# balaji1312/cassnat_asr_public

Measured on AMD Instinct MI355X. Metric: utterances_per_sec, higher is better.
Workload: dtype bf16; 1 GPU; BASELINE configs[1]: CASS-NAT 12L-enc / 1+3+2 dec blocks, d_model 256, 4 heads, d_ff 2048, V 5000, greedy NAST; 32 utterances x 1000 frames x 80 fbank per GPU per step; batch_per_gpu=32, frames=1000, feat_dim=80, global_batch=32, parallelism=utterance-sharded x1, decode_pipelines_per_gpu=2, batches_per_engine_pass=10, utterances_per_engine_pass=320, row_predictions=208, row_predictions_missed=0

## Files before the change

### cassnat_asr_public_amd/csrc/chain.hip

```cpp
#include <cstdio>
#include <cstdlib>
#include <algorithm>
#include <cmath>
#include <cstring>
#include <vector>

#include "kernels.h"

constexpr int CH_D = 256;
constexpr int CH_UNIT_BYTES = 16384;
constexpr int CH_RING = 8;
constexpr int CH_TAB_FLOATS = 5120;
constexpr int CH_TAB_BYTES = CH_TAB_FLOATS * 4;
constexpr int CH_LDS = CH_TAB_BYTES + CH_RING * CH_UNIT_BYTES;
static_assert(CH_LDS <= 160 * 1024, "LDS budget");
constexpr int CT_BO = 0, CT_LN1A = 256, CT_LN1B = 512, CT_B2 = 768, CT_NLNA = 1024, CT_NLNB = 1280, CT_BT = 1536,
              CT_B1 = 3072;
constexpr int CH_MAX_TAIL = 48, CH_MAX_FFN_TILES = 64;

__device__ long long ch_stamps[16];

typedef unsigned u32x4 __attribute__((ext_vector_type(4)));
typedef int v4i __attribute__((ext_vector_type(4)));
typedef int v8i __attribute__((ext_vector_type(8)));

struct ChainParams {
    float* x;
    const bf16* ctx;
    int ldctx;
    const uint4* wstream;
    const float* tab;
    bf16* out;
    int ldo;
    bf16* ln_out;
    int ld_ln;
    int M, ffn_tiles, tail_tiles, has_next;
    float eps;
    int stamps;
    int stamp_block;
    int x_in_blk, x_out_blk, store_x;
    int out_blk;
    int ctx_blk;
    const int* f8_q;
};

#define CH_STR2(x) #x
#define CH_STR(x) CH_STR2(x)
#define CH_DMA(src, dst)                                                                              \
    __builtin_amdgcn_global_load_lds((const __attribute__((address_space(1))) void*)(src),          \
                                     (__attribute__((address_space(3))) void*)(dst), 16, 0, 0)
#define CH_READ8(F, addr, OFFK)                                                                       \
    asm volatile("ds_read_b128 %0, %8 offset:" CH_STR(((OFFK) + 0) * 1024) "\n\t"                     \
                 "ds_read_b128 %1, %8 offset:" CH_STR(((OFFK) + 1) * 1024) "\n\t"                     \
                 "ds_read_b128 %2, %8 offset:" CH_STR(((OFFK) + 2) * 1024) "\n\t"                     \
                 "ds_read_b128 %3, %8 offset:" CH_STR(((OFFK) + 3) * 1024) "\n\t"                     \
                 "ds_read_b128 %4, %8 offset:" CH_STR(((OFFK) + 4) * 1024) "\n\t"                     \
                 "ds_read_b128 %5, %8 offset:" CH_STR(((OFFK) + 5) * 1024) "\n\t"                     \
                 "ds_read_b128 %6, %8 offset:" CH_STR(((OFFK) + 6) * 1024) "\n\t"                     \
                 "ds_read_b128 %7, %8 offset:" CH_STR(((OFFK) + 7) * 1024)                            \
                 : "=&v"(F[0]), "=&v"(F[1]), "=&v"(F[2]), "=&v"(F[3]), "=&v"(F[4]), "=&v"(F[5]),      \
                   "=&v"(F[6]), "=&v"(F[7])                                                           \
                 : "v"(addr)                                                                          \
                 : "memory")
#define CH_WAIT8(F)                                                                                   \
    asm volatile("s_waitcnt lgkmcnt(0)"                                                               \
                 : "+v"(F[0]), "+v"(F[1]), "+v"(F[2]), "+v"(F[3]), "+v"(F[4]), "+v"(F[5]), "+v"(F[6]), "+v"(F[7]) \
                 :: "memory")
__device__ __forceinline__ void ch_tab4_nowait(unsigned addr, f32x4& a, f32x4& b, f32x4& c, f32x4& d) {
    asm volatile("ds_read_b128 %0, %4\n\t"
                 "ds_read_b128 %1, %4 offset:32\n\t"
                 "ds_read_b128 %2, %4 offset:64\n\t"
                 "ds_read_b128 %3, %4 offset:96"
                 : "=&v"(a), "=&v"(b), "=&v"(c), "=&v"(d)
                 : "v"(addr)
                 : "memory");
}
template <typename D>
__device__ __forceinline__ void ch_tab4_nowait_after(unsigned addr, const D& dep, f32x4& a, f32x4& b, f32x4& c, f32x4& d) {
    asm volatile("ds_read_b128 %0, %4\n\t"
                 "ds_read_b128 %1, %4 offset:32\n\t"
                 "ds_read_b128 %2, %4 offset:64\n\t"
                 "ds_read_b128 %3, %4 offset:96"
                 : "=&v"(a), "=&v"(b), "=&v"(c), "=&v"(d)
                 : "v"(addr), "v"(dep)
                 : "memory");
}
template <typename D>
__device__ __forceinline__ void ch_tab4(unsigned addr, const D& dep, f32x4& a, f32x4& b, f32x4& c, f32x4& d) {
    asm volatile("ds_read_b128 %0, %4\n\t"
                 "ds_read_b128 %1, %4 offset:32\n\t"
                 "ds_read_b128 %2, %4 offset:64\n\t"
                 "ds_read_b128 %3, %4 offset:96\n\t"
                 "s_waitcnt lgkmcnt(0)"
                 : "=&v"(a), "=&v"(b), "=&v"(c), "=&v"(d)
                 : "v"(addr), "v"(dep)
                 : "memory");
}

#define CH_SB0_ __builtin_amdgcn_sched_barrier(0)
#define CH_LGKM_WAIT4(N, a, b, c, d) asm volatile("s_waitcnt lgkmcnt(" #N ")" : "+v"(a), "+v"(b), "+v"(c), "+v"(d) :: "memory")

template <bool ADD>
__device__ __forceinline__ void ch_layernorm_pack(f32x16 (&acc)[8], unsigned tab_lane, int off_a, int off_b, int off_add,
                                                  float eps, bf16x8 (&bop)[16]) {
    float s = 0.f;
#pragma unroll
    for (int nt = 0; nt < 8; ++nt)
#pragma unroll
        for (int r = 0; r < 16; ++r) s += acc[nt][r];
    s += __shfl_xor(s, 32);
    const float mean = s / (float)CH_D;
    float ss = 0.f;
#pragma unroll
    for (int nt = 0; nt < 8; ++nt)
#pragma unroll
        for (int r = 0; r < 16; ++r) ss = fmaf(acc[nt][r] - mean, acc[nt][r] - mean, ss);
    ss += __shfl_xor(ss, 32);
    const float inv = 1.0f / (sqrtf(ss / (float)(CH_D - 1)) + eps);
    f32x4 ga[2][4], be[2][4], ad[2][4];
    CH_SB0_;
    ch_tab4_nowait_after(tab_lane + off_a * 4, inv, ga[0][0], ga[0][1], ga[0][2], ga[0][3]);
    ch_tab4_nowait(tab_lane + off_b * 4, be[0][0], be[0][1], be[0][2], be[0][3]);
    if constexpr (ADD) ch_tab4_nowait(tab_lane + off_add * 4, ad[0][0], ad[0][1], ad[0][2], ad[0][3]);
#pragma unroll
    for (int nt = 0; nt < 8; ++nt) {
        const int c = nt & 1, n = c ^ 1;
        if (nt + 1 < 8) {
            ch_tab4_nowait(tab_lane + (off_a + 32 * (nt + 1)) * 4, ga[n][0], ga[n][1], ga[n][2], ga[n][3]);
            ch_tab4_nowait(tab_lane + (off_b + 32 * (nt + 1)) * 4, be[n][0], be[n][1], be[n][2], be[n][3]);
            if constexpr (ADD) ch_tab4_nowait(tab_lane + (off_add + 32 * (nt + 1)) * 4, ad[n][0], ad[n][1], ad[n][2], ad[n][3]);
            if constexpr (ADD) {
                CH_LGKM_WAIT4(12, ga[c][0], ga[c][1], ga[c][2], ga[c][3]);
                CH_LGKM_WAIT4(12, be[c][0], be[c][1], be[c][2], be[c][3]);
                CH_LGKM_WAIT4(12, ad[c][0], ad[c][1], ad[c][2], ad[c][3]);
            } else {
                CH_LGKM_WAIT4(8, ga[c][0], ga[c][1], ga[c][2], ga[c][3]);
                CH_LGKM_WAIT4(8, be[c][0], be[c][1], be[c][2], be[c][3]);
            }
        } else {
            CH_LGKM_WAIT4(0, ga[c][0], ga[c][1], ga[c][2], ga[c][3]);
            CH_LGKM_WAIT4(0, be[c][0], be[c][1], be[c][2], be[c][3]);
            if constexpr (ADD) CH_LGKM_WAIT4(0, ad[c][0], ad[c][1], ad[c][2], ad[c][3]);
        }
#pragma unroll
        for (int g = 0; g < 4; ++g)
#pragma unroll
            for (int e = 0; e < 4; ++e) {
                const int r = 4 * g + e;
                bop[2 * nt + (r >> 3)][r & 7] = (bf16)fmaf(ga[c][g][e] * (acc[nt][r] - mean), inv, be[c][g][e]);
                if constexpr (ADD) acc[nt][r] += ad[c][g][e];
            }
        asm volatile("" : "+v"(bop[2 * nt]), "+v"(bop[2 * nt + 1]));
        if constexpr (ADD) asm volatile("" : "+a"(acc[nt]));
    }
}

__device__ __forceinline__ void ch_add_channel(f32x16 (&acc)[8], unsigned tab_lane, int off) {
    f32x4 b[2][4];
    ch_tab4_nowait(tab_lane + off * 4, b[0][0], b[0][1], b[0][2], b[0][3]);
#pragma unroll
    for (int nt = 0; nt < 8; ++nt) {
        const int c = nt & 1, n = c ^ 1;
        if (nt + 1 < 8) {
            ch_tab4_nowait(tab_lane + (off + 32 * (nt + 1)) * 4, b[n][0], b[n][1], b[n][2], b[n][3]);
            CH_LGKM_WAIT4(4, b[c][0], b[c][1], b[c][2], b[c][3]);
        } else {
            CH_LGKM_WAIT4(0, b[c][0], b[c][1], b[c][2], b[c][3]);
        }
#pragma unroll
        for (int g = 0; g < 4; ++g)
#pragma unroll
            for (int e = 0; e < 4; ++e) acc[nt][4 * g + e] += b[c][g][e];
        asm volatile("" : "+a"(acc[nt]));
    }
}

template <int XS, int CS, bool CTX>
__device__ __forceinline__ void ch_load_rows(f32x4 (&xr)[32], bf16x8 (&bop)[16], const float* const (&xb)[8], const bf16* const (&cb)[4]) {
    if constexpr (CTX) {
        asm volatile("global_load_dwordx4 %[x0], %[xb0], off\n\t"
                     "global_load_dwordx4 %[x1], %[xb0], off offset:%[xo1]\n\t"
                     "global_load_dwordx4 %[x2], %[xb0], off offset:%[xo2]\n\t"
                     "global_load_dwordx4 %[x3], %[xb0], off offset:%[xo3]\n\t"
                     "global_load_dwordx4 %[x4], %[xb1], off\n\t"
                     "global_load_dwordx4 %[x5], %[xb1], off offset:%[xo1]\n\t"
                     "global_load_dwordx4 %[x6], %[xb1], off offset:%[xo2]\n\t"
                     "global_load_dwordx4 %[x7], %[xb1], off offset:%[xo3]\n\t"
                     "global_load_dwordx4 %[x8], %[xb2], off\n\t"
                     "global_load_dwordx4 %[x9], %[xb2], off offset:%[xo1]\n\t"
                     "global_load_dwordx4 %[x10], %[xb2], off offset:%[xo2]\n\t"
                     "global_load_dwordx4 %[x11], %[xb2], off offset:%[xo3]\n\t"
                     "global_load_dwordx4 %[x12], %[xb3], off\n\t"
                     "global_load_dwordx4 %[x13], %[xb3], off offset:%[xo1]\n\t"
                     "global_load_dwordx4 %[x14], %[xb3], off offset:%[xo2]\n\t"
                     "global_load_dwordx4 %[x15], %[xb3], off offset:%[xo3]\n\t"
                     "global_load_dwordx4 %[x16], %[xb4], off\n\t"
                     "global_load_dwordx4 %[x17], %[xb4], off offset:%[xo1]\n\t"
                     "global_load_dwordx4 %[x18], %[xb4], off offset:%[xo2]\n\t"
                     "global_load_dwordx4 %[x19], %[xb4], off offset:%[xo3]\n\t"
                     "global_load_dwordx4 %[x20], %[xb5], off\n\t"
                     "global_load_dwordx4 %[x21], %[xb5], off offset:%[xo1]\n\t"
                     "global_load_dwordx4 %[x22], %[xb5], off offset:%[xo2]\n\t"
                     "global_load_dwordx4 %[x23], %[xb5], off offset:%[xo3]\n\t"
                     "global_load_dwordx4 %[x24], %[xb6], off\n\t"
                     "global_load_dwordx4 %[x25], %[xb6], off offset:%[xo1]\n\t"
                     "global_load_dwordx4 %[x26], %[xb6], off offset:%[xo2]\n\t"
                     "global_load_dwordx4 %[x27], %[xb6], off offset:%[xo3]\n\t"
                     "global_load_dwordx4 %[x28], %[xb7], off\n\t"
                     "global_load_dwordx4 %[x29], %[xb7], off offset:%[xo1]\n\t"
                     "global_load_dwordx4 %[x30], %[xb7], off offset:%[xo2]\n\t"
                     "global_load_dwordx4 %[x31], %[xb7], off offset:%[xo3]\n\t"
                     "global_load_dwordx4 %[c0], %[cb0], off\n\t"
                     "global_load_dwordx4 %[c1], %[cb0], off offset:%[co1]\n\t"
                     "global_load_dwordx4 %[c2], %[cb0], off offset:%[co2]\n\t"
                     "global_load_dwordx4 %[c3], %[cb0], off offset:%[co3]\n\t"
                     "global_load_dwordx4 %[c4], %[cb1], off\n\t"
                     "global_load_dwordx4 %[c5], %[cb1], off offset:%[co1]\n\t"
                     "global_load_dwordx4 %[c6], %[cb1], off offset:%[co2]\n\t"
                     "global_load_dwordx4 %[c7], %[cb1], off offset:%[co3]\n\t"
                     "global_load_dwordx4 %[c8], %[cb2], off\n\t"
                     "global_load_dwordx4 %[c9], %[cb2], off offset:%[co1]\n\t"
                     "global_load_dwordx4 %[c10], %[cb2], off offset:%[co2]\n\t"
                     "global_load_dwordx4 %[c11], %[cb2], off offset:%[co3]\n\t"
                     "global_load_dwordx4 %[c12], %[cb3], off\n\t"
                     "global_load_dwordx4 %[c13], %[cb3], off offset:%[co1]\n\t"
                     "global_load_dwordx4 %[c14], %[cb3], off offset:%[co2]\n\t"
                     "global_load_dwordx4 %[c15], %[cb3], off offset:%[co3]\n\t"
                     "s_waitcnt vmcnt(0)"
                     : [x0] "=&a"(xr[0]), [x1] "=&a"(xr[1]), [x2] "=&a"(xr[2]), [x3] "=&a"(xr[3]), [x4] "=&a"(xr[4]), [x5] "=&a"(xr[5]), [x6] "=&a"(xr[6]), [x7] "=&a"(xr[7]), [x8] "=&a"(xr[8]), [x9] "=&a"(xr[9]), [x10] "=&a"(xr[10]), [x11] "=&a"(xr[11]), [x12] "=&a"(xr[12]), [x13] "=&a"(xr[13]), [x14] "=&a"(xr[14]), [x15] "=&a"(xr[15]), [x16] "=&a"(xr[16]), [x17] "=&a"(xr[17]), [x18] "=&a"(xr[18]), [x19] "=&a"(xr[19]), [x20] "=&a"(xr[20]), [x21] "=&a"(xr[21]), [x22] "=&a"(xr[22]), [x23] "=&a"(xr[23]), [x24] "=&a"(xr[24]), [x25] "=&a"(xr[25]), [x26] "=&a"(xr[26]), [x27] "=&a"(xr[27]), [x28] "=&a"(xr[28]), [x29] "=&a"(xr[29]), [x30] "=&a"(xr[30]), [x31] "=&a"(xr[31]), [c0] "=&v"(bop[0]), [c1] "=&v"(bop[1]), [c2] "=&v"(bop[2]), [c3] "=&v"(bop[3]), [c4] "=&v"(bop[4]), [c5] "=&v"(bop[5]), [c6] "=&v"(bop[6]), [c7] "=&v"(bop[7]), [c8] "=&v"(bop[8]), [c9] "=&v"(bop[9]), [c10] "=&v"(bop[10]), [c11] "=&v"(bop[11]), [c12] "=&v"(bop[12]), [c13] "=&v"(bop[13]), [c14] "=&v"(bop[14]), [c15] "=&v"(bop[15])
                     : [xb0] "v"(xb[0]), [xb1] "v"(xb[1]), [xb2] "v"(xb[2]), [xb3] "v"(xb[3]), [xb4] "v"(xb[4]), [xb5] "v"(xb[5]), [xb6] "v"(xb[6]), [xb7] "v"(xb[7]), [cb0] "v"(cb[0]), [cb1] "v"(cb[1]), [cb2] "v"(cb[2]), [cb3] "v"(cb[3])
                       , [xo1] "n"(XS), [xo2] "n"(2 * XS), [xo3] "n"(3 * XS), [co1] "n"(CS), [co2] "n"(2 * CS), [co3] "n"(3 * CS)
                     : "memory");
    } else {
        asm volatile("global_load_dwordx4 %[x0], %[xb0], off\n\t"
                     "global_load_dwordx4 %[x1], %[xb0], off offset:%[xo1]\n\t"
                     "global_load_dwordx4 %[x2], %[xb0], off offset:%[xo2]\n\t"
                     "global_load_dwordx4 %[x3], %[xb0], off offset:%[xo3]\n\t"
                     "global_load_dwordx4 %[x4], %[xb1], off\n\t"
                     "global_load_dwordx4 %[x5], %[xb1], off offset:%[xo1]\n\t"
                     "global_load_dwordx4 %[x6], %[xb1], off offset:%[xo2]\n\t"
                     "global_load_dwordx4 %[x7], %[xb1], off offset:%[xo3]\n\t"
                     "global_load_dwordx4 %[x8], %[xb2], off\n\t"
                     "global_load_dwordx4 %[x9], %[xb2], off offset:%[xo1]\n\t"
                     "global_load_dwordx4 %[x10], %[xb2], off offset:%[xo2]\n\t"
                     "global_load_dwordx4 %[x11], %[xb2], off offset:%[xo3]\n\t"
                     "global_load_dwordx4 %[x12], %[xb3], off\n\t"
                     "global_load_dwordx4 %[x13], %[xb3], off offset:%[xo1]\n\t"
                     "global_load_dwordx4 %[x14], %[xb3], off offset:%[xo2]\n\t"
                     "global_load_dwordx4 %[x15], %[xb3], off offset:%[xo3]\n\t"
                     "global_load_dwordx4 %[x16], %[xb4], off\n\t"
                     "global_load_dwordx4 %[x17], %[xb4], off offset:%[xo1]\n\t"
                     "global_load_dwordx4 %[x18], %[xb4], off offset:%[xo2]\n\t"
                     "global_load_dwordx4 %[x19], %[xb4], off offset:%[xo3]\n\t"
                     "global_load_dwordx4 %[x20], %[xb5], off\n\t"
                     "global_load_dwordx4 %[x21], %[xb5], off offset:%[xo1]\n\t"
                     "global_load_dwordx4 %[x22], %[xb5], off offset:%[xo2]\n\t"
                     "global_load_dwordx4 %[x23], %[xb5], off offset:%[xo3]\n\t"
                     "global_load_dwordx4 %[x24], %[xb6], off\n\t"
                     "global_load_dwordx4 %[x25], %[xb6], off offset:%[xo1]\n\t"
                     "global_load_dwordx4 %[x26], %[xb6], off offset:%[xo2]\n\t"
                     "global_load_dwordx4 %[x27], %[xb6], off offset:%[xo3]\n\t"
                     "global_load_dwordx4 %[x28], %[xb7], off\n\t"
                     "global_load_dwordx4 %[x29], %[xb7], off offset:%[xo1]\n\t"
                     "global_load_dwordx4 %[x30], %[xb7], off offset:%[xo2]\n\t"
                     "global_load_dwordx4 %[x31], %[xb7], off offset:%[xo3]\n\t"
                     "s_waitcnt vmcnt(0)"
                     : [x0] "=&a"(xr[0]), [x1] "=&a"(xr[1]), [x2] "=&a"(xr[2]), [x3] "=&a"(xr[3]), [x4] "=&a"(xr[4]), [x5] "=&a"(xr[5]), [x6] "=&a"(xr[6]), [x7] "=&a"(xr[7]), [x8] "=&a"(xr[8]), [x9] "=&a"(xr[9]), [x10] "=&a"(xr[10]), [x11] "=&a"(xr[11]), [x12] "=&a"(xr[12]), [x13] "=&a"(xr[13]), [x14] "=&a"(xr[14]), [x15] "=&a"(xr[15]), [x16] "=&a"(xr[16]), [x17] "=&a"(xr[17]), [x18] "=&a"(xr[18]), [x19] "=&a"(xr[19]), [x20] "=&a"(xr[20]), [x21] "=&a"(xr[21]), [x22] "=&a"(xr[22]), [x23] "=&a"(xr[23]), [x24] "=&a"(xr[24]), [x25] "=&a"(xr[25]), [x26] "=&a"(xr[26]), [x27] "=&a"(xr[27]), [x28] "=&a"(xr[28]), [x29] "=&a"(xr[29]), [x30] "=&a"(xr[30]), [x31] "=&a"(xr[31])
                     : [xb0] "v"(xb[0]), [xb1] "v"(xb[1]), [xb2] "v"(xb[2]), [xb3] "v"(xb[3]), [xb4] "v"(xb[4]), [xb5] "v"(xb[5]), [xb6] "v"(xb[6]), [xb7] "v"(xb[7])
                       , [xo1] "n"(XS), [xo2] "n"(2 * XS), [xo3] "n"(3 * XS)
                     : "memory");
    }
}

__device__ __forceinline__ void ch_layernorm_pack8(f32x16 (&acc)[8], unsigned tab_lane, int off_a, int off_b, int off_add,
                                                   float eps, v4i (&b8)[8]) {
    float s = 0.f;
#pragma unroll
    for (int nt = 0; nt < 8; ++nt)
#pragma unroll
        for (int r = 0; r < 16; ++r) s += acc[nt][r];
    s += __shfl_xor(s, 32);
    const float mean = s / (float)CH_D;
    float ss = 0.f;
#pragma unroll
    for (int nt = 0; nt < 8; ++nt)
#pragma unroll
        for (int r = 0; r < 16; ++r) ss = fmaf(acc[nt][r] - mean, acc[nt][r] - mean, ss);
    ss += __shfl_xor(ss, 32);
    const float inv = 1.0f / (sqrtf(ss / (float)(CH_D - 1)) + eps);
    f32x4 ga[2][4], be[2][4], ad[2][4];
    CH_SB0_;
    ch_tab4_nowait_after(tab_lane + off_a * 4, inv, ga[0][0], ga[0][1], ga[0][2], ga[0][3]);
    ch_tab4_nowait(tab_lane + off_b * 4, be[0][0], be[0][1], be[0][2], be[0][3]);
    ch_tab4_nowait(tab_lane + off_add * 4, ad[0][0], ad[0][1], ad[0][2], ad[0][3]);
#pragma unroll
    for (int nt = 0; nt < 8; ++nt) {
        const int c = nt & 1, n = c ^ 1;
        if (nt + 1 < 8) {
            ch_tab4_nowait(tab_lane + (off_a + 32 * (nt + 1)) * 4, ga[n][0], ga[n][1], ga[n][2], ga[n][3]);
            ch_tab4_nowait(tab_lane + (off_b + 32 * (nt + 1)) * 4, be[n][0], be[n][1], be[n][2], be[n][3]);
            ch_tab4_nowait(tab_lane + (off_add + 32 * (nt + 1)) * 4, ad[n][0], ad[n][1], ad[n][2], ad[n][3]);
            CH_LGKM_WAIT4(12, ga[c][0], ga[c][1], ga[c][2], ga[c][3]);
            CH_LGKM_WAIT4(12, be[c][0], be[c][1], be[c][2], be[c][3]);
            CH_LGKM_WAIT4(12, ad[c][0], ad[c][1], ad[c][2], ad[c][3]);
        } else {
            CH_LGKM_WAIT4(0, ga[c][0], ga[c][1], ga[c][2], ga[c][3]);
            CH_LGKM_WAIT4(0, be[c][0], be[c][1], be[c][2], be[c][3]);
            CH_LGKM_WAIT4(0, ad[c][0], ad[c][1], ad[c][2], ad[c][3]);
        }
#pragma unroll
        for (int g = 0; g < 4; ++g) {
            float v[4];
#pragma unroll
            for (int e = 0; e < 4; ++e) {
                v[e] = __builtin_amdgcn_fmed3f(fmaf(ga[c][g][e] * (acc[nt][4 * g + e] - mean), inv, be[c][g][e]), -448.f, 448.f);
                acc[nt][4 * g + e] += ad[c][g][e];
            }
            b8[nt][g] = __builtin_amdgcn_cvt_pk_fp8_f32(v[0], v[1], b8[nt][g], false);
            b8[nt][g] = __builtin_amdgcn_cvt_pk_fp8_f32(v[2], v[3], b8[nt][g], true);
        }
        asm volatile("" : "+v"(b8[nt]));
        asm volatile("" : "+a"(acc[nt]));
    }
}

#define CH_LAND_FRAGMENTS(EXTRA)                                                                                \
    asm volatile(EXTRA "s_waitcnt lgkmcnt(0)"                                                                  \
                 : "+v"(Fa[0]), "+v"(Fa[1]), "+v"(Fa[2]), "+v"(Fa[3]), "+v"(Fa[4]), "+v"(Fa[5]), "+v"(Fa[6]), "+v"(Fa[7]),     \
                   "+v"(Fb[0]), "+v"(Fb[1]), "+v"(Fb[2]), "+v"(Fb[3]), "+v"(Fb[4]), "+v"(Fb[5]), "+v"(Fb[6]), "+v"(Fb[7])      \
                 :: "memory")

#define CH_MF CN_MFMA16_ASM
#define CH_DRAIN "s_nop 13\n\t"
#define CH_NODRAIN ""
#ifdef CH_EXP_NO_READ
#define CH_RD2(n0, n1, K) ""
#else
#define CH_RD2(n0, n1, K) "ds_read_b128 %[" #n0 "], %[ra] offset:" CH_STR((K) * 1024) "\n\t"                   \
                          "ds_read_b128 %[" #n1 "], %[ra] offset:" CH_STR(((K) + 1) * 1024) "\n\t"
#endif
#define CH_PRE_A "s_waitcnt lgkmcnt(0)\n\t"
#define CH_PRE_A4 "s_waitcnt lgkmcnt(4)\n\t"
#define CH_PRE_BO(M0OFF) "s_add_u32 m0, %[m0w], " CH_STR(M0OFF) "\n\ts_waitcnt lgkmcnt(0)\n\t"
#ifdef CH_EXP_NO_BARRIER
#define CH_PRE_BE(M0OFF) CH_PRE_BO(M0OFF)
#else
#define CH_PRE_BE(M0OFF) "s_waitcnt vmcnt(16)\n\ts_barrier\n\ts_add_u32 m0, %[m0w], " CH_STR(M0OFF) "\n\ts_waitcnt lgkmcnt(0)\n\t"
#endif
#define CH_PRE_B_0 CH_PRE_BE
#define CH_PRE_B_1 CH_PRE_BO
#define CH_PRE_B_2 CH_PRE_BE
#define CH_PRE_B_3 CH_PRE_BO
#define CH_PRE_B_4 CH_PRE_BE
#define CH_PRE_B_5 CH_PRE_BO
#define CH_PRE_B_6 CH_PRE_BE
#define CH_PRE_B_7 CH_PRE_BO
#ifdef CH_EXP_NO_DMA
#define CH_DMA0(SOFF) "v_add_u32 %[tv], " CH_STR(SOFF) ", %[vo]\n\t"
#define CH_DMA1 ""
#define CH_DMA2 ""
#define CH_DMA3 ""
#else
#define CH_DMA0(SOFF) "v_add_u32 %[tv], " CH_STR(SOFF) ", %[vo]\n\tglobal_load_lds_dwordx4 %[tv], %[sb]\n\t"
#define CH_DMA1 "global_load_lds_dwordx4 %[tv], %[sb] offset:1024\n\t"
#define CH_DMA2 "global_load_lds_dwordx4 %[tv], %[sb] offset:2048\n\t"
#define CH_DMA3 "global_load_lds_dwordx4 %[tv], %[sb] offset:3072\n\t"
#endif
#define CH_BLK1(CIO, CC, C0, acc, Fc, B, BO, Fn, RA, RK, PRE, D0, D1, D2, D3, SB, POST)                        \
    asm volatile(PRE                                                                                           \
                 CH_MF "%[c], %[f0], %[b0], " C0 "\n\t" CH_RD2(n0, n1, (RK) + 0)                               \
                 CH_MF "%[c], %[f1], %[b1], %[c]\n\t" CH_RD2(n2, n3, (RK) + 2)                                 \
                 CH_MF "%[c], %[f2], %[b2], %[c]\n\t" CH_RD2(n4, n5, (RK) + 4)                                 \
                 CH_MF "%[c], %[f3], %[b3], %[c]\n\t" CH_RD2(n6, n7, (RK) + 6)                                 \
                 CH_MF "%[c], %[f4], %[b4], %[c]\n\t" D0                                                       \
                 CH_MF "%[c], %[f5], %[b5], %[c]\n\t" D1                                                       \
                 CH_MF "%[c], %[f6], %[b6], %[c]\n\t" D2                                                       \
                 CH_MF "%[c], %[f7], %[b7], %[c]\n\t" D3 POST                                                  \
                 : [c] CIO CC(acc), [n0] "=&v"(Fn[0]), [n1] "=&v"(Fn[1]), [n2] "=&v"(Fn[2]), [n3] "=&v"(Fn[3]), \
                   [n4] "=&v"(Fn[4]), [n5] "=&v"(Fn[5]), [n6] "=&v"(Fn[6]), [n7] "=&v"(Fn[7]), [tv] "=&v"(tv)  \
                 : [f0] "v"(Fc[0]), [f1] "v"(Fc[1]), [f2] "v"(Fc[2]), [f3] "v"(Fc[3]), [f4] "v"(Fc[4]),        \
                   [f5] "v"(Fc[5]), [f6] "v"(Fc[6]), [f7] "v"(Fc[7]), [b0] "v"(B[(BO) + 0]), [b1] "v"(B[(BO) + 1]), \
                   [b2] "v"(B[(BO) + 2]), [b3] "v"(B[(BO) + 3]), [b4] "v"(B[(BO) + 4]), [b5] "v"(B[(BO) + 5]), \
                   [b6] "v"(B[(BO) + 6]), [b7] "v"(B[(BO) + 7]), [ra] "v"(RA), [m0w] "s"(m0_wave), [vo] "v"(voff), \
                   [sb] "s"(SB)                                                                                \
                 : "memory", "scc")
#define CH_BLK1A(K, acc, Fc, B, BO, Fn, RA, RK, PRE, D0, D1, D2, D3, SB, POST)                                 \
    asm volatile(PRE                                                                                           \
                 CH_MF "%[c" #K "], %[f0], %[b0], %[c" #K "]\n\t" CH_RD2(n0, n1, (RK) + 0)                       \
                 CH_MF "%[c" #K "], %[f1], %[b1], %[c" #K "]\n\t" CH_RD2(n2, n3, (RK) + 2)                       \
                 CH_MF "%[c" #K "], %[f2], %[b2], %[c" #K "]\n\t" CH_RD2(n4, n5, (RK) + 4)                       \
                 CH_MF "%[c" #K "], %[f3], %[b3], %[c" #K "]\n\t" CH_RD2(n6, n7, (RK) + 6)                       \
                 CH_MF "%[c" #K "], %[f4], %[b4], %[c" #K "]\n\t" D0                                           \
                 CH_MF "%[c" #K "], %[f5], %[b5], %[c" #K "]\n\t" D1                                           \
                 CH_MF "%[c" #K "], %[f6], %[b6], %[c" #K "]\n\t" D2                                           \
                 CH_MF "%[c" #K "], %[f7], %[b7], %[c" #K "]\n\t" D3 POST                                      \
                 : [c0] "+a"(acc[0]), [c1] "+a"(acc[1]), [c2] "+a"(acc[2]), [c3] "+a"(acc[3]), [c4] "+a"(acc[4]), \
                   [c5] "+a"(acc[5]), [c6] "+a"(acc[6]), [c7] "+a"(acc[7]), [n0] "=&v"(Fn[0]), [n1] "=&v"(Fn[1]), \
                   [n2] "=&v"(Fn[2]), [n3] "=&v"(Fn[3]), [n4] "=&v"(Fn[4]), [n5] "=&v"(Fn[5]), [n6] "=&v"(Fn[6]), \
                   [n7] "=&v"(Fn[7]), [tv] "=&v"(tv)                                                           \
                 : [f0] "v"(Fc[0]), [f1] "v"(Fc[1]), [f2] "v"(Fc[2]), [f3] "v"(Fc[3]), [f4] "v"(Fc[4]),        \
                   [f5] "v"(Fc[5]), [f6] "v"(Fc[6]), [f7] "v"(Fc[7]), [b0] "v"(B[(BO) + 0]), [b1] "v"(B[(BO) + 1]), \
                   [b2] "v"(B[(BO) + 2]), [b3] "v"(B[(BO) + 3]), [b4] "v"(B[(BO) + 4]), [b5] "v"(B[(BO) + 5]), \
                   [b6] "v"(B[(BO) + 6]), [b7] "v"(B[(BO) + 7]), [ra] "v"(RA), [m0w] "s"(m0_wave), [vo] "v"(voff), \
                   [sb] "s"(SB)                                                                                \
                 : "memory", "scc")
#define CH_BLK2(acc, Fc, pbv, Fn, RA, RK, PRE, D0, D1, D2, D3, SB, POST)                                       \
    asm volatile(PRE                                                                                           \
                 CH_MF "%[c0], %[f0], %[pb], %[c0]\n\t" CH_RD2(n0, n1, (RK) + 0)                               \
                 CH_MF "%[c1], %[f1], %[pb], %[c1]\n\t" CH_RD2(n2, n3, (RK) + 2)                               \
                 CH_MF "%[c2], %[f2], %[pb], %[c2]\n\t" CH_RD2(n4, n5, (RK) + 4)                               \
                 CH_MF "%[c3], %[f3], %[pb], %[c3]\n\t" CH_RD2(n6, n7, (RK) + 6)                               \
                 CH_MF "%[c4], %[f4], %[pb], %[c4]\n\t" D0                                                     \
                 CH_MF "%[c5], %[f5], %[pb], %[c5]\n\t" D1                                                     \
                 CH_MF "%[c6], %[f6], %[pb], %[c6]\n\t" D2                                                     \
                 CH_MF "%[c7], %[f7], %[pb], %[c7]\n\t" D3 POST                                                \
                 : [c0] "+a"(acc[0]), [c1] "+a"(acc[1]), [c2] "+a"(acc[2]), [c3] "+a"(acc[3]), [c4] "+a"(acc[4]), \
                   [c5] "+a"(acc[5]), [c6] "+a"(acc[6]), [c7] "+a"(acc[7]), [n0] "=&v"(Fn[0]), [n1] "=&v"(Fn[1]), \
                   [n2] "=&v"(Fn[2]), [n3] "=&v"(Fn[3]), [n4] "=&v"(Fn[4]), [n5] "=&v"(Fn[5]), [n6] "=&v"(Fn[6]), \
                   [n7] "=&v"(Fn[7]), [tv] "=&v"(tv)                                                           \
                 : [f0] "v"(Fc[0]), [f1] "v"(Fc[1]), [f2] "v"(Fc[2]), [f3] "v"(Fc[3]), [f4] "v"(Fc[4]),        \
                   [f5] "v"(Fc[5]), [f6] "v"(Fc[6]), [f7] "v"(Fc[7]), [pb] "v"(pbv), [ra] "v"(RA),             \
                   [m0w] "s"(m0_wave), [vo] "v"(voff), [sb] "s"(SB)                                            \
                 : "memory", "scc")
#define CH_M1R(PRE, X, F, B, N0, N1, RA, K)                                                                    \
    asm volatile(PRE CH_MF "%[c], %[f], %[b], %[c]\n\t" CH_RD2(n0, n1, K)                                      \
                 : [c] "+v"(X), [n0] "=&v"(N0), [n1] "=&v"(N1)                                                 \
                 : [f] "v"(F), [b] "v"(B), [ra] "v"(RA)                                                        \
                 : "memory")
#define CH_M1(X, F, B) asm volatile(CH_MF "%[c], %[f], %[b], %[c]" : [c] "+v"(X) : [f] "v"(F), [b] "v"(B) : "memory")
#define CH_SB0 __builtin_amdgcn_sched_barrier(0)

#define CH8_MF "v_mfma_scale_f32_32x32x64_f8f6f4 "
#define CH8_SC ", %[qa], %[qb] op_sel_hi:[0,0,0]\n\t"
#define CH8_DRAIN "s_nop 15\n\ts_nop 4\n\t"
#define CH8_JOIN(lo, hi) __builtin_shufflevector(__builtin_bit_cast(v4i, lo), __builtin_bit_cast(v4i, hi), 0, 1, 2, 3, 4, 5, 6, 7)
#define CH8_A(F, t) CH8_JOIN(F[2 * (t)], F[2 * (t) + 1])
#define CH8_M1R(PRE, X, A, B, N0, N1, N2, N3, RA, K, QA, QB)                                                   \
    asm volatile(PRE CH8_MF "%[c], %[a], %[b], %[c]" CH8_SC CH_RD2(n0, n1, K) CH_RD2(n2, n3, (K) + 2)          \
                 : [c] "+v"(X), [n0] "=&v"(N0), [n1] "=&v"(N1), [n2] "=&v"(N2), [n3] "=&v"(N3)                 \
                 : [a] "v"(A), [b] "v"(B), [ra] "v"(RA), [qa] "v"(QA), [qb] "v"(QB), [m0w] "s"(m0_wave)         \
                 : "memory", "scc")
#define CH8_M1(X, A, B, QA, QB)                                                                                \
    asm volatile(CH8_MF "%[c], %[a], %[b], %[c]" CH8_SC : [c] "+v"(X) : [a] "v"(A), [b] "v"(B), [qa] "v"(QA), [qb] "v"(QB) : "memory")
#define CH8_M1D(M0OFF, X, A, B, D0, D1, SB, QA, QB)                                                            \
    asm volatile("s_add_u32 m0, %[m0w], " CH_STR(M0OFF) "\n\t" CH8_MF "%[c], %[a], %[b], %[c]" CH8_SC D0 D1    \
                 : [c] "+v"(X), [tv] "+v"(tv)                                                                  \
                 : [a] "v"(A), [b] "v"(B), [qa] "v"(QA), [qb] "v"(QB), [vo] "v"(voff), [sb] "s"(SB),            \
                   [m0w] "s"(m0_wave)                                                                          \
                 : "memory", "scc")
#define CH8_BLK2(acc, C0, C1, C2, C3, A0, A1, A2, A3, HB, Fn, RA, RK, PRE, D0, D1, D2, D3, SB, POST, QA, QB)    \
    asm volatile(PRE                                                                                           \
                 CH8_MF "%[" #C0 "], %[a0], %[hb], %[" #C0 "]" CH8_SC CH_RD2(n0, n1, (RK) + 0) CH_RD2(n2, n3, (RK) + 2) \
                 CH8_MF "%[" #C1 "], %[a1], %[hb], %[" #C1 "]" CH8_SC CH_RD2(n4, n5, (RK) + 4) CH_RD2(n6, n7, (RK) + 6) \
                 CH8_MF "%[" #C2 "], %[a2], %[hb], %[" #C2 "]" CH8_SC D0 D1                                    \
                 CH8_MF "%[" #C3 "], %[a3], %[hb], %[" #C3 "]" CH8_SC D2 D3 POST                               \
                 : [c0] "+a"(acc[0]), [c1] "+a"(acc[1]), [c2] "+a"(acc[2]), [c3] "+a"(acc[3]), [c4] "+a"(acc[4]), \
                   [c5] "+a"(acc[5]), [c6] "+a"(acc[6]), [c7] "+a"(acc[7]), [n0] "=&v"(Fn[0]), [n1] "=&v"(Fn[1]), \
                   [n2] "=&v"(Fn[2]), [n3] "=&v"(Fn[3]), [n4] "=&v"(Fn[4]), [n5] "=&v"(Fn[5]), [n6] "=&v"(Fn[6]), \
                   [n7] "=&v"(Fn[7]), [tv] "=&v"(tv)                                                           \
                 : [a0] "v"(A0), [a1] "v"(A1), [a2] "v"(A2), [a3] "v"(A3), [hb] "v"(HB), [ra] "v"(RA),         \
                   [m0w] "s"(m0_wave), [vo] "v"(voff), [sb] "s"(SB), [qa] "v"(QA), [qb] "v"(QB)                \
                 : "memory", "scc")

#define CH_POSITIONS(X)                                                                                        \
    X(0, ra0, 8, ra0, 16, 0x1C000, 0x1C000, sb_cur)  X(1, ra0, 24, ra0, 32, 0x0, 0x0, sb_next)                 \
    X(2, ra0, 40, ra0, 48, 0x4000, 0x4000, sb_next)  X(3, ra0, 56, ra1, 0, 0x8000, 0x8000, sb_next)            \
    X(4, ra1, 8, ra1, 16, 0xC000, 0xC000, sb_next)   X(5, ra1, 24, ra1, 32, 0x10000, 0x10000, sb_next)         \
    X(6, ra1, 40, ra1, 48, 0x14000, 0x14000, sb_next) X(7, ra1, 56, ra0, 0, 0x18000, 0x18000, sb_next)

template <bool SWISH, bool F8>
__global__ __launch_bounds__(256) void chain_kernel(ChainParams p) {
    extern __shared__ __attribute__((aligned(16))) unsigned char smem[];
    const int tid = threadIdx.x, lane = tid & 63;
    const int wave = __builtin_amdgcn_readfirstlane(tid >> 6);
    const int half = lane >> 5, l31 = lane & 31;
    const int m = blockIdx.x * 128 + 32 * wave + l31;
    const int mc = m < p.M ? m : p.M - 1;
    const bool live = m < p.M;
#define CH_STAMP(i)                                                                              \
    if (p.stamps && (int)blockIdx.x == p.stamp_block && tid == 0) ch_stamps[i] = (long long)__builtin_amdgcn_s_memtime();
    CH_STAMP(0)
    if (p.stamps && (int)blockIdx.x == p.stamp_block && tid == 0) ch_stamps[10] = (long long)__builtin_amdgcn_s_memrealtime();
    const int G_OUT = p.ctx ? 1 : 0, G_FFN = F8 ? p.ffn_tiles >> 3 : p.ffn_tiles >> 2, G_TAIL = p.tail_tiles >> 3;
    const int NG = G_OUT + G_FFN + G_TAIL;
#ifdef CH_ROTATE
    const int rotg = G_FFN ? (int)((blockIdx.x * 5u) % (unsigned)G_FFN) : 0;
#else
    const int rotg = 0;
#endif
    unsigned char* ring = smem + CH_TAB_BYTES;
    auto ffn_group = [&](int g) -> int { return g + rotg >= G_FFN ? g + rotg - G_FFN : g + rotg; };
    auto group_base = [&](int g) -> const uint4* {
        if (g > NG - 1) g = NG - 1;
        if (g >= G_OUT && g < G_OUT + G_FFN) g = G_OUT + ffn_group(g - G_OUT);
        return p.wstream + (long long)g * 8 * 1024;
    };

    f32x4 xr[32];
    bf16x8 bop[16];
    const int rb = blockIdx.x * 4 + wave, nrb = (p.M + 31) >> 5;
    {
        const uint4* ts = reinterpret_cast<const uint4*>(p.tab) + 5 * wave * 64 + lane;
#pragma unroll
        for (int j = 0; j < 5; ++j) CH_DMA(ts + j * 64, smem + (5 * wave + j) * 1024);
    }
    if (NG > 0) {
        const uint4* g0 = group_base(0);
        for (int u = 0; u < CH_RING - 1; ++u) {
            const uint4* src = g0 + ((long long)u * 16 + 4 * wave) * 64 + lane;
            unsigned char* dst = ring + u * CH_UNIT_BYTES + 4 * wave * 1024;
#pragma unroll
            for (int j = 0; j < 4; ++j) CH_DMA(src + j * 64, dst + j * 1024);
        }
    }
    {
#ifdef CH_EXP_HOT_X
        const float* xp = p.x + (long long)wave * 8192 + 4 * lane;
#else
        const float* xp = p.x_in_blk ? p.x + (long long)(rb < nrb ? rb : nrb - 1) * 8192 + 4 * lane
                                     : p.x + (long long)mc * CH_D + 4 * half;
#endif
        const int step = p.x_in_blk ? 256 : 8;
        const float* xb[8];
#pragma unroll
        for (int nt = 0; nt < 8; ++nt) xb[nt] = xp + step * 4 * nt;
        const bf16* cp = !p.ctx ? nullptr
                         : p.ctx_blk ? p.ctx + ((long long)(rb < nrb ? rb : nrb - 1) * 16 * 64 + lane) * 8
                                     : p.ctx + (long long)mc * p.ldctx + 8 * half;
        const int cstep = p.ctx_blk ? 512 : 16;
        const bf16* cb[4];
#pragma unroll
        for (int q = 0; q < 4; ++q) cb[q] = cp + cstep * 4 * q;
        if (!p.ctx) {
            if (p.x_in_blk) ch_load_rows<1024, 32, false>(xr, bop, xb, cb);
            else ch_load_rows<32, 32, false>(xr, bop, xb, cb);
        } else if (p.x_in_blk) {
            if (p.ctx_blk) ch_load_rows<1024, 1024, true>(xr, bop, xb, cb);
            else ch_load_rows<1024, 32, true>(xr, bop, xb, cb);
        } else {
            if (p.ctx_blk) ch_load_rows<32, 1024, true>(xr, bop, xb, cb);
            else ch_load_rows<32, 32, true>(xr, bop, xb, cb);
        }
    }

    f32x16 acc[8];
#pragma unroll
    for (int nt = 0; nt < 8; ++nt)
#pragma unroll
        for (int g = 0; g < 4; ++g)
#pragma unroll
            for (int e = 0; e < 4; ++e) acc[nt][4 * g + e] = xr[4 * nt + g][e];
    CH_STAMP(1)

    const unsigned ring_lds = (unsigned)(size_t)(__attribute__((address_space(3))) unsigned char*)ring;
    const unsigned ra0 = ring_lds + lane * 16, ra1 = ra0 + 4 * CH_UNIT_BYTES;
    const unsigned tab_lane = (unsigned)(size_t)(__attribute__((address_space(3))) unsigned char*)(smem + 16 * half);
    const unsigned voff = (unsigned)(lane * 16 + wave * 4096);
    const unsigned m0_wave = __builtin_amdgcn_readfirstlane(ring_lds + wave * 4096);
    unsigned tv = 0;

    bf16x8 Fa[8], Fb[8];
    asm volatile("s_waitcnt vmcnt(0)\n\ts_barrier" ::: "memory");
    CH_STAMP(2)
    int gpos = 0;

    if (p.ctx) {
        const uint4* sb_cur = group_base(gpos);
        const uint4* sb_next = group_base(gpos + 1);
#define CH_S1(k, RA_A, RK_A, RA_B, RK_B, M0OFF, SOFF, SB)                                                     \
        CH_BLK1A(k, acc, Fa, bop, 0, Fb, RA_A, RK_A, CH_PRE_A, "", "", "", "", SB, CH_NODRAIN);                \
        CH_BLK1A(k, acc, Fb, bop, 8, Fa, RA_B, RK_B, CH_PRE_B_##k(M0OFF), CH_DMA0(SOFF), CH_DMA1, CH_DMA2, CH_DMA3, SB, CH_NODRAIN);
        CH_READ8(Fa, ra0, 0);
        CH_WAIT8(Fa);
        asm volatile("s_nop 1" ::: "memory");
        CH_POSITIONS(CH_S1)
#undef CH_S1
        CH_LAND_FRAGMENTS("");
        asm volatile(CH_DRAIN : "+a"(acc[0]), "+a"(acc[1]), "+a"(acc[2]), "+a"(acc[3]), "+a"(acc[4]), "+a"(acc[5]),
                     "+a"(acc[6]), "+a"(acc[7]) :: "memory");
        ++gpos;
        ch_add_channel(acc, tab_lane, CT_BO);
    }
    CH_STAMP(3)

    if constexpr (F8) {
      if (p.ffn_tiles) {
        v4i b8[8] = {};
        ch_layernorm_pack8(acc, tab_lane, CT_LN1A, CT_LN1B, CT_B2, p.eps, b8);
        CH_STAMP(4)
        const int NP = p.ffn_tiles >> 1;
        f32x16 xa0, xb0, xa1, xb1;
        f32x4 b1v[8];
        v8i hid8 = {};
        const int qa1 = p.f8_q[0], qb1 = p.f8_q[1], qa2 = p.f8_q[2], qb2 = p.f8_q[3];
        auto tabp = [&](int pp) -> unsigned { return tab_lane + (unsigned)((CT_B1 + 64 * (pp < NP ? pp : NP - 1)) * 4); };
#define CH8_TAB8(addr)                                                                                         \
        ch_tab4_nowait(addr, b1v[0], b1v[1], b1v[2], b1v[3]);                                                  \
        ch_tab4_nowait((addr) + 128, b1v[4], b1v[5], b1v[6], b1v[7]);
#define CH8_B(kk) CH8_JOIN(b8[2 * (kk)], b8[2 * (kk) + 1])
        CH8_TAB8(tabp(0))
        CH_READ8(Fa, ra0, 0);
        asm volatile("s_waitcnt lgkmcnt(0)" : "+v"(b1v[0]), "+v"(b1v[1]), "+v"(b1v[2]), "+v"(b1v[3]), "+v"(b1v[4]), "+v"(b1v[5]),
                     "+v"(b1v[6]), "+v"(b1v[7]), "+v"(Fa[0]), "+v"(Fa[1]), "+v"(Fa[2]), "+v"(Fa[3]), "+v"(Fa[4]), "+v"(Fa[5]),
                     "+v"(Fa[6]), "+v"(Fa[7]) :: "memory");
#define CH8_ACT_PIECE(XA, XB, i)                                                                               \
        {                                                                                                      \
            const float v0_ = __builtin_amdgcn_fmed3f(((i) < 4 ? XA : XB)[4 * ((i) & 3) + 0], 0.f, 448.f);     \
            const float v1_ = __builtin_amdgcn_fmed3f(((i) < 4 ? XA : XB)[4 * ((i) & 3) + 1], 0.f, 448.f);     \
            const float v2_ = __builtin_amdgcn_fmed3f(((i) < 4 ? XA : XB)[4 * ((i) & 3) + 2], 0.f, 448.f);     \
            const float v3_ = __builtin_amdgcn_fmed3f(((i) < 4 ? XA : XB)[4 * ((i) & 3) + 3], 0.f, 448.f);     \
            hid8[i] = __builtin_amdgcn_cvt_pk_fp8_f32(v0_, v1_, hid8[i], false);                               \
            hid8[i] = __builtin_amdgcn_cvt_pk_fp8_f32(v2_, v3_, hid8[i], true);                                \
            asm volatile("" : "+v"(hid8));                                                                     \
        }
#define CH8_ACT_GAP(HAS_OLD, XA, XB, i)                                                                        \
        CH_SB0;                                                                                                \
        if constexpr (HAS_OLD) CH8_ACT_PIECE(XA, XB, i)                                                        \
        CH_SB0;
#define CH8_BIAS16(lo) __builtin_shufflevector(__builtin_shufflevector(b1v[lo], b1v[(lo) + 1], 0, 1, 2, 3, 4, 5, 6, 7),   \
                                               __builtin_shufflevector(b1v[(lo) + 2], b1v[(lo) + 3], 0, 1, 2, 3, 4, 5, 6, 7), \
                                               0, 1, 2, 3, 4, 5, 6, 7, 8, 9, 10, 11, 12, 13, 14, 15)
#define CH8_W1N(k, RA_A, RK_A, RA_B, RK_B, M0OFF, SOFF, SB, XNA, XNB, XOA, XOB, HAS_OLD, PNEXT)                 \
        XNA = CH8_BIAS16(0);                                                                                   \
        XNB = CH8_BIAS16(4);                                                                                   \
        CH8_M1R(CH_PRE_A, XNA, CH8_A(Fa, 0), CH8_B(0), Fb[0], Fb[1], Fb[2], Fb[3], RA_A, (RK_A) + 0, qa1, qb1); \
        CH8_ACT_GAP(HAS_OLD, XOA, XOB, 0)                                                                      \
        CH8_M1R("", XNA, CH8_A(Fa, 1), CH8_B(1), Fb[4], Fb[5], Fb[6], Fb[7], RA_A, (RK_A) + 4, qa1, qb1);      \
        CH8_ACT_GAP(HAS_OLD, XOA, XOB, 1)                                                                      \
        CH8_M1(XNA, CH8_A(Fa, 2), CH8_B(2), qa1, qb1);                                                         \
        CH8_ACT_GAP(HAS_OLD, XOA, XOB, 2)                                                                      \
        CH8_M1(XNA, CH8_A(Fa, 3), CH8_B(3), qa1, qb1);                                                         \
        CH8_ACT_GAP(HAS_OLD, XOA, XOB, 3)                                                                      \
        CH8_M1R(CH_PRE_B_##k(M0OFF), XNB, CH8_A(Fb, 0), CH8_B(0), Fa[0], Fa[1], Fa[2], Fa[3], RA_B, (RK_B) + 0, qa1, qb1); \
        CH8_ACT_GAP(HAS_OLD, XOA, XOB, 4)                                                                      \
        CH8_M1R("", XNB, CH8_A(Fb, 1), CH8_B(1), Fa[4], Fa[5], Fa[6], Fa[7], RA_B, (RK_B) + 4, qa1, qb1);      \
        CH8_ACT_GAP(HAS_OLD, XOA, XOB, 5)                                                                      \
        CH8_M1D(M0OFF, XNB, CH8_A(Fb, 2), CH8_B(2), CH_DMA0(SOFF), CH_DMA1, SB, qa1, qb1);                            \
        CH8_ACT_GAP(HAS_OLD, XOA, XOB, 6)                                                                      \
        CH8_M1D(M0OFF, XNB, CH8_A(Fb, 3), CH8_B(3), CH_DMA2, CH_DMA3, SB, qa1, qb1);                                  \
        CH8_ACT_GAP(HAS_OLD, XOA, XOB, 7)                                                                      \
        CH8_TAB8(tabp(PNEXT))
#define CH8_PRE_A8 "s_waitcnt lgkmcnt(8)\n\t"
#define CH8_W2N(k, RA_A, RK_A, RA_B, RK_B, M0OFF, SOFF, SB, PREA, POST)                                        \
        CH8_BLK2(acc, c0, c1, c2, c3, CH8_A(Fa, 0), CH8_A(Fa, 1), CH8_A(Fa, 2), CH8_A(Fa, 3), hid8, Fb, RA_A, RK_A, PREA, "", "", \
                 "", "", SB, CH_NODRAIN, qa2, qb2);                                                            \
        CH8_BLK2(acc, c4, c5, c6, c7, CH8_A(Fb, 0), CH8_A(Fb, 1), CH8_A(Fb, 2), CH8_A(Fb, 3), hid8, Fa, RA_B, RK_B,              \
                 CH_PRE_B_##k(M0OFF), CH_DMA0(SOFF), CH_DMA1, CH_DMA2, CH_DMA3, SB, POST, qa2, qb2);
#define CH8_FFN_GROUP(FIRST, LAST)                                                                             \
        {                                                                                                      \
            const uint4* sb_cur = group_base(gpos);                                                            \
            const uint4* sb_next = group_base(gpos + 1);                                                       \
            const int t0 = 4 * g;                                                                              \
            if constexpr (FIRST) {                                                                             \
                CH8_W1N(0, ra0, 8, ra0, 16, 0x1C000, 0x1C000, sb_cur, xa0, xb0, xa1, xb1, false, 1)            \
                             \
                asm volatile(CH8_DRAIN "s_waitcnt lgkmcnt(0)" : "+v"(xa0), "+v"(xb0), "+v"(b1v[0]), "+v"(b1v[1]), "+v"(b1v[2]), \
                             "+v"(b1v[3]), "+v"(b1v[4]), "+v"(b1v[5]), "+v"(b1v[6]), "+v"(b1v[7]), "+v"(Fa[0]), "+v"(Fa[1]),     \
                             "+v"(Fa[2]), "+v"(Fa[3]), "+v"(Fa[4]), "+v"(Fa[5]), "+v"(Fa[6]), "+v"(Fa[7]) :: "memory");          \
            } else {                                                                                           \
                CH8_W2N(0, ra0, 8, ra0, 16, 0x1C000, 0x1C000, sb_cur, CH8_PRE_A8, CH_NODRAIN)                  \
            }                                                                                                  \
            CH8_W1N(1, ra0, 24, ra0, 32, 0x0, 0x0, sb_next, xa1, xb1, xa0, xb0, true, t0 + 2)                  \
            CH8_W2N(2, ra0, 40, ra0, 48, 0x4000, 0x4000, sb_next, CH8_PRE_A8, CH_NODRAIN)                      \
            CH8_W1N(3, ra0, 56, ra1, 0, 0x8000, 0x8000, sb_next, xa0, xb0, xa1, xb1, true, t0 + 3)             \
            CH8_W2N(4, ra1, 8, ra1, 16, 0xC000, 0xC000, sb_next, CH8_PRE_A8, CH_NODRAIN)                       \
            CH8_W1N(5, ra1, 24, ra1, 32, 0x10000, 0x10000, sb_next, xa1, xb1, xa0, xb0, true, t0 + 4)          \
            CH8_W2N(6, ra1, 40, ra1, 48, 0x14000, 0x14000, sb_next, CH8_PRE_A8, CH_NODRAIN)                    \
            if constexpr (!(LAST)) {                                                                           \
                CH8_W1N(7, ra1, 56, ra0, 0, 0x18000, 0x18000, sb_next, xa0, xb0, xa1, xb1, true, t0 + 5)       \
            } else {                                                                                           \
                               \
                asm volatile("" : "+v"(xa1), "+v"(xb1));                                                       \
                CH_SB0;                                                                                        \
                CH8_ACT_PIECE(xa1, xb1, 0) CH8_ACT_PIECE(xa1, xb1, 1) CH8_ACT_PIECE(xa1, xb1, 2) CH8_ACT_PIECE(xa1, xb1, 3) \
                CH8_ACT_PIECE(xa1, xb1, 4) CH8_ACT_PIECE(xa1, xb1, 5) CH8_ACT_PIECE(xa1, xb1, 6) CH8_ACT_PIECE(xa1, xb1, 7) \
                CH_SB0;                                                                                        \
                CH8_W2N(7, ra1, 56, ra0, 0, 0x18000, 0x18000, sb_next, CH_PRE_A, CH8_DRAIN "s_waitcnt lgkmcnt(0)\n\t") \
            }                                                                                                  \
            ++g;                                                                                               \
            ++gpos;                                                                                            \
        }
        int g = 0;
        if (G_FFN == 1) {
            CH8_FFN_GROUP(true, true)
        } else {
            CH8_FFN_GROUP(true, false)
            while (g < G_FFN - 1) CH8_FFN_GROUP(false, false)
            CH8_FFN_GROUP(false, true)
        }
#undef CH8_FFN_GROUP
#undef CH8_W1N
#undef CH8_W2N
#undef CH8_ACT_GAP
#undef CH8_ACT_PIECE
        CH_LAND_FRAGMENTS("");
        asm volatile("s_waitcnt lgkmcnt(0)" : "+v"(b1v[0]), "+v"(b1v[1]), "+v"(b1v[2]), "+v"(b1v[3]), "+v"(b1v[4]), "+v"(b1v[5]),
                     "+v"(b1v[6]), "+v"(b1v[7]) :: "memory");
      }
    } else
    if (p.ffn_tiles) {
        ch_layernorm_pack<true>(acc, tab_lane, CT_LN1A, CT_LN1B, CT_B2, p.eps, bop);
        CH_STAMP(4)
        const int NTL = p.ffn_tiles;
        f32x16 xh0, xh1;
        f32x4 b1v[4];
        bf16x8 pb[2];
        auto tabb = [&](int t) -> unsigned { return tab_lane + (unsigned)((CT_B1 + 32 * (t < NTL ? t : NTL - 1)) * 4); };
        ch_tab4_nowait(tabb(0), b1v[0], b1v[1], b1v[2], b1v[3]);
        CH_READ8(Fa, ra0, 0);
        asm volatile("s_waitcnt lgkmcnt(0)" : "+v"(b1v[0]), "+v"(b1v[1]), "+v"(b1v[2]), "+v"(b1v[3]), "+v"(Fa[0]), "+v"(Fa[1]), "+v"(Fa[2]),
                     "+v"(Fa[3]), "+v"(Fa[4]), "+v"(Fa[5]), "+v"(Fa[6]), "+v"(Fa[7]) :: "memory");
#define CH_ACT_PIECE(XO, i)                                                                                    \
        {                                                                                                      \
            if constexpr (SWISH) {                                                                             \
                const float v0_ = XO[2 * (i)], v1_ = XO[2 * (i) + 1];                                          \
                pb[(i) >> 2][2 * ((i) & 3)] = (bf16)(v0_ * (1.f / (1.f + __expf(-v0_))));                      \
                pb[(i) >> 2][2 * ((i) & 3) + 1] = (bf16)(v1_ * (1.f / (1.f + __expf(-v1_))));                  \
            } else {                                                                                           \
                const int b0_ = __float_as_int(XO[2 * (i)]), b1_ = __float_as_int(XO[2 * (i) + 1]);            \
                pb[(i) >> 2][2 * ((i) & 3)] = (bf16)__int_as_float(b0_ > 0 ? b0_ : 0);                         \
                pb[(i) >> 2][2 * ((i) & 3) + 1] = (bf16)__int_as_float(b1_ > 0 ? b1_ : 0);                     \
            }                                                                                                  \
            asm volatile("" : "+v"(pb[(i) >> 2]));   \
        }
#define CH_ACT_GAP(HAS_OLD, XO, i)                                                                             \
        CH_SB0;                                                                                                \
        if constexpr (HAS_OLD) CH_ACT_PIECE(XO, i)                                                             \
        CH_SB0;
#define CH_W1N(k, RA_A, RK_A, RA_B, RK_B, M0OFF, SOFF, SB, XN, XO, HAS_OLD, TNEXT)                             \
        XN = __builtin_shufflevector(__builtin_shufflevector(b1v[0], b1v[1], 0, 1, 2, 3, 4, 5, 6, 7),          \
                                     __builtin_shufflevector(b1v[2], b1v[3], 0, 1, 2, 3, 4, 5, 6, 7),          \
                                     0, 1, 2, 3, 4, 5, 6, 7, 8, 9, 10, 11, 12, 13, 14, 15);                   \
        CH_M1R(CH_PRE_A, XN, Fa[0], bop[0], Fb[0], Fb[1], RA_A, (RK_A) + 0);                                   \
        CH_ACT_GAP(HAS_OLD, XO, 0)                                                                             \
        CH_M1R("", XN, Fa[1], bop[1], Fb[2], Fb[3], RA_A, (RK_A) + 2);                                         \
        CH_ACT_GAP(HAS_OLD, XO, 1)                                                                             \
        CH_M1R("", XN, Fa[2], bop[2], Fb[4], Fb[5], RA_A, (RK_A) + 4);                                         \
        CH_ACT_GAP(HAS_OLD, XO, 2)                                                                             \
        CH_M1R("", XN, Fa[3], bop[3], Fb[6], Fb[7], RA_A, (RK_A) + 6);                                         \
        CH_ACT_GAP(HAS_OLD, XO, 3)                                                                             \
        CH_M1(XN, Fa[4], bop[4]);                                                                              \
        CH_ACT_GAP(HAS_OLD, XO, 4)                                                                             \
        CH_M1(XN, Fa[5], bop[5]);                                                                              \
        CH_ACT_GAP(HAS_OLD, XO, 5)                                                                             \
        CH_M1(XN, Fa[6], bop[6]);                                                                              \
        CH_ACT_GAP(HAS_OLD, XO, 6)                                                                             \
        CH_M1(XN, Fa[7], bop[7]);                                                                              \
        CH_ACT_GAP(HAS_OLD, XO, 7)                                                                             \
        CH_BLK1("+", "v", "%[c]", XN, Fb, bop, 8, Fa, RA_B, RK_B, CH_PRE_B_##k(M0OFF), CH_DMA0(SOFF), CH_DMA1, CH_DMA2, \
                CH_DMA3, SB, CH_NODRAIN);                                                                      \
        ch_tab4_nowait(tabb(TNEXT), b1v[0], b1v[1], b1v[2], b1v[3]);
#define CH_W2N(k, RA_A, RK_A, RA_B, RK_B, M0OFF, SOFF, SB, PREA, POST)                                        \
        CH_BLK2(acc, Fa, pb[0], Fb, RA_A, RK_A, PREA, "", "", "", "", SB, CH_NODRAIN);                         \
        CH_BLK2(acc, Fb, pb[1], Fa, RA_B, RK_B, CH_PRE_B_##k(M0OFF), CH_DMA0(SOFF), CH_DMA1, CH_DMA2, CH_DMA3, SB, POST);
#define CH_FFN_GROUP(FIRST, LAST)                                                                              \
        {                                                                                                      \
            const uint4* sb_cur = group_base(gpos);                                                            \
            const uint4* sb_next = group_base(gpos + 1);                                                       \
            const int t0 = 4 * g;                                                                              \
            if constexpr (FIRST) {                                                                             \
                CH_W1N(0, ra0, 8, ra0, 16, 0x1C000, 0x1C000, sb_cur, xh0, xh1, false, 1)                       \
                 \
                 \
                 \
                asm volatile("s_nop 13\n\ts_nop 13\n\ts_waitcnt lgkmcnt(0)" : "+v"(xh0), "+v"(b1v[0]), "+v"(b1v[1]), "+v"(b1v[2]), "+v"(b1v[3]), "+v"(Fa[0]), \
                             "+v"(Fa[1]), "+v"(Fa[2]), "+v"(Fa[3]), "+v"(Fa[4]), "+v"(Fa[5]), "+v"(Fa[6]), "+v"(Fa[7]) :: "memory"); \
            } else {                                                                                           \
                CH_W2N(0, ra0, 8, ra0, 16, 0x1C000, 0x1C000, sb_cur, CH_PRE_A4, CH_NODRAIN)                    \
            }                                                                                                  \
            CH_W1N(1, ra0, 24, ra0, 32, 0x0, 0x0, sb_next, xh1, xh0, true, t0 + 2)                             \
            CH_W2N(2, ra0, 40, ra0, 48, 0x4000, 0x4000, sb_next, CH_PRE_A4, CH_NODRAIN)                        \
            CH_W1N(3, ra0, 56, ra1, 0, 0x8000, 0x8000, sb_next, xh0, xh1, true, t0 + 3)                        \
            CH_W2N(4, ra1, 8, ra1, 16, 0xC000, 0xC000, sb_next, CH_PRE_A4, CH_NODRAIN)                         \
            CH_W1N(5, ra1, 24, ra1, 32, 0x10000, 0x10000, sb_next, xh1, xh0, true, t0 + 4)                     \
            CH_W2N(6, ra1, 40, ra1, 48, 0x14000, 0x14000, sb_next, CH_PRE_A4, CH_NODRAIN)                      \
            if constexpr (!(LAST)) {                                                                           \
                CH_W1N(7, ra1, 56, ra0, 0, 0x18000, 0x18000, sb_next, xh0, xh1, true, t0 + 5)                  \
            } else {                                                                                           \
                 \
                 \
                 \
                asm volatile("" : "+v"(xh1));                                                                  \
                CH_SB0;                                                                                        \
                _Pragma("unroll") for (int i = 0; i < 8; ++i) CH_ACT_PIECE(xh1, i)                             \
                CH_SB0;                                                                                        \
                CH_W2N(7, ra1, 56, ra0, 0, 0x18000, 0x18000, sb_next, CH_PRE_A, CH_DRAIN "s_waitcnt lgkmcnt(0)\n\t") \
            }                                                                                                  \
            ++g;                                                                                               \
            ++gpos;                                                                                            \
        }
        int g = 0;
        if (G_FFN == 1) {
            CH_FFN_GROUP(true, true)
        } else {
            CH_FFN_GROUP(true, false)
            while (g < G_FFN - 1) CH_FFN_GROUP(false, false)
            CH_FFN_GROUP(false, true)
        }
#undef CH_FFN_GROUP
#undef CH_W1N
#undef CH_W2N
#undef CH_ACT_GAP
#undef CH_ACT_PIECE
        CH_LAND_FRAGMENTS("");
        asm volatile("s_waitcnt lgkmcnt(0)" : "+v"(b1v[0]), "+v"(b1v[1]), "+v"(b1v[2]), "+v"(b1v[3]) :: "memory");
    }
    CH_STAMP(5)

    if (p.store_x && (p.x_out_blk ? rb < nrb : live)) {
        float* xp = p.x_out_blk ? p.x + (long long)rb * 8192 + 4 * lane : p.x + (long long)m * CH_D + 4 * half;
        const int step = p.x_out_blk ? 256 : 8;
#pragma unroll
        for (int nt = 0; nt < 8; ++nt)
#pragma unroll
            for (int g = 0; g < 4; ++g) {
                f32x4 o;
#pragma unroll
                for (int e = 0; e < 4; ++e) o[e] = acc[nt][4 * g + e];
                *reinterpret_cast<f32x4*>(xp + step * (4 * nt + g)) = o;
            }
    }
    CH_STAMP(6)
    if (p.has_next) {
        ch_layernorm_pack<false>(acc, tab_lane, CT_NLNA, CT_NLNB, 0, p.eps, bop);
        CH_STAMP(7)
        if (p.ln_out) {
            if (live) {
                bf16* op = p.ln_out + (long long)m * p.ld_ln + 4 * half;
#pragma unroll
                for (int k = 0; k < 16; ++k)
#pragma unroll
                    for (int q = 0; q < 2; ++q) {
                        bf16x4 o;
#pragma unroll
                        for (int e = 0; e < 4; ++e) o[e] = bop[k][4 * q + e];
                        *reinterpret_cast<bf16x4*>(op + 16 * k + 8 * q) = o;
                    }
            }
        }
        if (G_TAIL > 0) {
            f32x16 q0, q1;
            f32x4 btv[4];
            bf16x4 o_[4];
            u32x4 w_[2];
            const int NTT = 8 * G_TAIL;
            auto tabt = [&](int tt) -> unsigned { return tab_lane + (unsigned)((CT_BT + 32 * (tt < NTT ? tt : NTT - 1)) * 4); };
            bf16* op16 = p.out + (long long)m * p.ldo + 8 * half;
            unsigned char* ob16 = reinterpret_cast<unsigned char*>(p.out) + (long long)rb * (p.ldo >> 5) * 2048 + lane * 16;
            unsigned char* st_base = p.out_blk ? ob16 : reinterpret_cast<unsigned char*>(op16);
            const int st_tile = p.out_blk ? 2048 : 64, st_half = p.out_blk ? 1024 : 32;
            const bool st_on = (p.out_blk ? rb < nrb : live) && p.stamps != 2;
            ch_tab4_nowait(tabt(0), btv[0], btv[1], btv[2], btv[3]);
            CH_READ8(Fa, ra0, 0);
            asm volatile("s_waitcnt lgkmcnt(0)" : "+v"(btv[0]), "+v"(btv[1]), "+v"(btv[2]), "+v"(btv[3]), "+v"(Fa[0]), "+v"(Fa[1]),
                         "+v"(Fa[2]), "+v"(Fa[3]), "+v"(Fa[4]), "+v"(Fa[5]), "+v"(Fa[6]), "+v"(Fa[7]) :: "memory");
#define CH_TAIL_STORE(v, ptr) *(ptr) = (v)
#define CH_EPI_CVT(QO, g0)                                                                                     \
            {                                                                                                  \
                _Pragma("unroll") for (int g_ = (g0); g_ < (g0) + 2; ++g_)                                     \
                    _Pragma("unroll") for (int e = 0; e < 4; ++e) o_[g_][e] = (bf16)QO[4 * g_ + e];             \
                asm volatile("" : "+v"(o_[g0]), "+v"(o_[(g0) + 1]));                                            \
            }
#define CH_EPI_OUT(TT, gp)                                                                                     \
            {                                                                                                  \
                const uint2 lo_ = __builtin_bit_cast(uint2, o_[2 * (gp)]), hi_ = __builtin_bit_cast(uint2, o_[2 * (gp) + 1]); \
                const auto s0_ = __builtin_amdgcn_permlane32_swap(lo_.x, hi_.x, false, false);                 \
                const auto s1_ = __builtin_amdgcn_permlane32_swap(lo_.y, hi_.y, false, false);                 \
                w_[gp] = u32x4{s0_[0], s1_[0], s0_[1], s1_[1]};                                                \
                if (st_on) CH_TAIL_STORE(w_[gp], reinterpret_cast<u32x4*>(st_base + (long long)(TT) * st_tile + (gp) * st_half)); \
                else asm volatile("" :: "v"(w_[gp]));                                                          \
            }
#define CH_EPI_GAP(HAS_OLD, CODE)                                                                              \
            CH_SB0;                                                                                            \
            if constexpr (HAS_OLD) CODE                                                                        \
            CH_SB0;
#define CH_S5N(k, RA_A, RK_A, RA_B, RK_B, M0OFF, SOFF, SB, QN, QO, HAS_OLD)                                    \
            QN = __builtin_shufflevector(__builtin_shufflevector(btv[0], btv[1], 0, 1, 2, 3, 4, 5, 6, 7),      \
                                         __builtin_shufflevector(btv[2], btv[3], 0, 1, 2, 3, 4, 5, 6, 7),      \
                                         0, 1, 2, 3, 4, 5, 6, 7, 8, 9, 10, 11, 12, 13, 14, 15);   \
            CH_M1R(CH_PRE_A, QN, Fa[0], bop[0], Fb[0], Fb[1], RA_A, (RK_A) + 0);                               \
            CH_SB0;                                                                                            \
            ch_tab4_nowait(tabt(8 * g + (k) + 1), btv[0], btv[1], btv[2], btv[3]);   \
            CH_SB0;                                                                                            \
            CH_M1R("", QN, Fa[1], bop[1], Fb[2], Fb[3], RA_A, (RK_A) + 2);                                     \
            CH_SB0;                                                                                            \
            CH_M1R("", QN, Fa[2], bop[2], Fb[4], Fb[5], RA_A, (RK_A) + 4);                                     \
            CH_EPI_GAP(HAS_OLD, CH_EPI_CVT(QO, 0))                                                             \
            CH_M1R("", QN, Fa[3], bop[3], Fb[6], Fb[7], RA_A, (RK_A) + 6);                                     \
            CH_EPI_GAP(HAS_OLD, CH_EPI_CVT(QO, 2))                                                             \
            CH_M1(QN, Fa[4], bop[4]);                                                                          \
            CH_EPI_GAP(HAS_OLD, CH_EPI_OUT(8 * g + (k) - 1, 0))                                                \
            CH_M1(QN, Fa[5], bop[5]);                                                                          \
            CH_EPI_GAP(HAS_OLD, CH_EPI_OUT(8 * g + (k) - 1, 1))                                                \
            CH_M1(QN, Fa[6], bop[6]);                                                                          \
            CH_SB0;                                                                                            \
            CH_M1(QN, Fa[7], bop[7]);                                                                          \
            CH_SB0;                                                                                            \
            CH_BLK1("+", "v", "%[c]", QN, Fb, bop, 8, Fa, RA_B, RK_B, CH_PRE_B_##k(M0OFF), CH_DMA0(SOFF), CH_DMA1, CH_DMA2, \
                    CH_DMA3, SB, CH_NODRAIN);
#define CH_TAIL_GROUP(FIRST, LAST)                                                                             \
            {                                                                                                  \
                const uint4* sb_cur = group_base(gpos);                                                        \
                const uint4* sb_next = group_base(gpos + 1);                                                   \
                CH_S5N(0, ra0, 8, ra0, 16, 0x1C000, 0x1C000, sb_cur, q0, q1, !(FIRST))                         \
                CH_S5N(1, ra0, 24, ra0, 32, 0x0, 0x0, sb_next, q1, q0, true)                                   \
                CH_S5N(2, ra0, 40, ra0, 48, 0x4000, 0x4000, sb_next, q0, q1, true)                             \
                CH_S5N(3, ra0, 56, ra1, 0, 0x8000, 0x8000, sb_next, q1, q0, true)                              \
                CH_S5N(4, ra1, 8, ra1, 16, 0xC000, 0xC000, sb_next, q0, q1, true)                              \
                CH_S5N(5, ra1, 24, ra1, 32, 0x10000, 0x10000, sb_next, q1, q0, true)                           \
                CH_S5N(6, ra1, 40, ra1, 48, 0x14000, 0x14000, sb_next, q0, q1, true)                           \
                CH_S5N(7, ra1, 56, ra0, 0, 0x18000, 0x18000, sb_next, q1, q0, true)                            \
                if constexpr (LAST) {                                                                          \
                       \
                    CH_LAND_FRAGMENTS("");                                                                     \
                    asm volatile(CH_DRAIN : "+v"(q1));                                                         \
                    CH_SB0;                                                                                    \
                    CH_EPI_CVT(q1, 0) CH_EPI_CVT(q1, 2) CH_EPI_OUT(8 * g + 7, 0) CH_EPI_OUT(8 * g + 7, 1)      \
                    CH_SB0;                                                                                    \
                }                                                                                              \
                ++g;                                                                                           \
                ++gpos;                                                                                        \
            }
            int g = 0;
            if (G_TAIL == 1) {
                CH_TAIL_GROUP(true, true)
            } else {
                CH_TAIL_GROUP(true, false)
                while (g < G_TAIL - 1) CH_TAIL_GROUP(false, false)
                CH_TAIL_GROUP(false, true)
            }
#undef CH_TAIL_GROUP
#undef CH_S5N
#undef CH_EPI_GAP
#undef CH_EPI_OUT
#undef CH_EPI_CVT
            CH_LAND_FRAGMENTS("");
            asm volatile("s_waitcnt lgkmcnt(0)" : "+v"(btv[0]), "+v"(btv[1]), "+v"(btv[2]), "+v"(btv[3]) :: "memory");
        }
    }
    CH_STAMP(8)
    asm volatile("s_waitcnt vmcnt(0) lgkmcnt(0)" ::: "memory");
    CH_STAMP(9)
    if (p.stamps && (int)blockIdx.x == p.stamp_block && tid == 0) ch_stamps[11] = (long long)__builtin_amdgcn_s_memrealtime();
}

int chain_print_stamps() {
    long long h[16];
    CN_HIP_CHECK(hipMemcpyFromSymbol(h, HIP_SYMBOL(ch_stamps), sizeof(h)));
    static const char* names[] = {"prologue issue", "x/ctx landed + acc", "first unit visible", "S1 out-proj", "LN1 + b2",
                                  "S3 ffn loop", "S4 x store", "LNn", "S5 tail", "drain"};
    for (int i = 1; i < 10; ++i) fprintf(stderr, "[chain stamps] %-20s %8lld ticks\n", names[i], h[i] - h[i - 1]);
    fprintf(stderr, "[chain stamps] total %lld ticks (s_memtime)\n", h[9] - h[0]);
    fprintf(stderr, "[chain stamps] wall %.2f us (s_memrealtime) -> %.0f MHz\n", (h[11] - h[10]) / 100.0,
            (double)(h[9] - h[0]) / ((h[11] - h[10]) / 100.0));
    return 0;
}

int launch_chain(const ChainArgs& a, hipStream_t s) {
    if (a.f8 && (a.swish || a.dff <= 0 || a.dff % 256 != 0 || !a.f8_q)) {
        cn_set_error("chain: the e4m3 feed-forward form needs d_ff % 256 == 0 and the ReLU activation");
        return -1;
    }
    if (a.d != CH_D || a.dff < 0 || a.dff % 128 != 0 || a.dff / 32 > CH_MAX_FFN_TILES || a.tail_n < 0 || a.tail_n % 256 != 0 ||
        a.tail_n / 32 > CH_MAX_TAIL || (a.tail_n > 0 && (!a.has_next || !a.out)) || (a.has_next && !a.out && !a.ln_out)) {
        cn_set_error("chain: needs d_model == 256, d_ff % 128 == 0 <= 2048, tail width % 256 == 0 <= 1536");
        return -1;
    }
    if (a.M <= 0) return 0;
    ChainParams p;
    p.x = a.x;
    p.ctx = reinterpret_cast<const bf16*>(a.ctx);
    p.ldctx = a.ldctx;
    p.wstream = reinterpret_cast<const uint4*>(a.wstream);
    p.tab = a.tab;
    p.out = reinterpret_cast<bf16*>(a.out);
    p.ldo = a.ldo;
    p.ln_out = reinterpret_cast<bf16*>(a.ln_out ? a.ln_out : (a.tail_n == 0 ? a.out : nullptr));
    p.ld_ln = a.ln_out ? a.ld_ln : a.ldo;
    p.M = a.M;
    p.ffn_tiles = a.dff / 32;
    p.tail_tiles = a.tail_n / 32;
    p.has_next = a.has_next;
    p.eps = a.eps;
    static const int stamps = cn_exp_env("CASSNAT_CHAIN_STAMPS") ? atoi(cn_exp_env("CASSNAT_CHAIN_STAMPS")) : 0;
    p.stamps = stamps;
    static const int stamp_block = cn_exp_env("CASSNAT_CHAIN_STAMP_BLOCK") ? atoi(cn_exp_env("CASSNAT_CHAIN_STAMP_BLOCK")) : 0;
    p.stamp_block = stamp_block;
    p.x_in_blk = a.x_in_blocked;
    p.x_out_blk = a.x_out_blocked;
    p.store_x = a.store_x && (a.ctx || a.dff);
    p.out_blk = a.out_blocked && a.tail_n > 0;
    p.ctx_blk = a.ctx && a.ctx_blocked;
    p.f8_q = a.f8_q;
    if (p.ctx_blk && a.ldctx != CH_D) {
        cn_set_error("chain: a blocked ctx has 256 columns");
        return -1;
    }
    if (p.out_blk && a.ldo % 32 != 0) {
        cn_set_error("chain: a blocked tail output needs ldo % 32 == 0");
        return -1;
    }
    static CnAttrOnce attr_once;
    int attr_dev;
    if (attr_once.need(&attr_dev)) {
        CN_HIP_CHECK(hipFuncSetAttribute((const void*)chain_kernel<false, false>, hipFuncAttributeMaxDynamicSharedMemorySize, CH_LDS));
        CN_HIP_CHECK(hipFuncSetAttribute((const void*)chain_kernel<true, false>, hipFuncAttributeMaxDynamicSharedMemorySize, CH_LDS));
        CN_HIP_CHECK(hipFuncSetAttribute((const void*)chain_kernel<false, true>, hipFuncAttributeMaxDynamicSharedMemorySize, CH_LDS));
        attr_once.mark(attr_dev);
    }
    if (a.f8)
        hipLaunchKernelGGL((chain_kernel<false, true>), dim3(cn_ceil_div(p.M, 128)), dim3(256), CH_LDS, s, p);
    else if (a.swish)
        hipLaunchKernelGGL((chain_kernel<true, false>), dim3(cn_ceil_div(p.M, 128)), dim3(256), CH_LDS, s, p);
    else
        hipLaunchKernelGGL((chain_kernel<false, false>), dim3(cn_ceil_div(p.M, 128)), dim3(256), CH_LDS, s, p);
    CN_HIP_CHECK(hipGetLastError());
    return 0;
}

static inline uint16_t ch_bf16_bits(float f) { return cn_host_op16(f); }

size_t chain_stream_units(int has_outproj, int dff, int tail_n, int f8) {
    return (has_outproj ? 8 : 0) + (f8 ? 1 : 2) * (dff / 32) + tail_n / 32;
}

static void ch_pack_rows(const float* w, int ld, int rt, bool acc_order, uint16_t* out) {
    for (int f = 0; f < 16; ++f)
        for (int lane = 0; lane < 64; ++lane)
            for (int j = 0; j < 8; ++j) {
                const int k = acc_order ? 32 * (f >> 1) + 16 * (f & 1) + 8 * (j >> 2) + 4 * (lane >> 5) + (j & 3)
                                        : 16 * f + 8 * (lane >> 5) + j;
                out[((size_t)f * 64 + lane) * 8 + j] = ch_bf16_bits(w[(size_t)(32 * rt + (lane & 31)) * ld + k]);
            }
}
static void ch_pack_w2(const float* w2, int dff, int t, uint16_t* out) {
    for (int s = 0; s < 2; ++s)
        for (int nt = 0; nt < 8; ++nt)
            for (int lane = 0; lane < 64; ++lane)
                for (int j = 0; j < 8; ++j)
                    out[((size_t)(8 * s + nt) * 64 + lane) * 8 + j] = ch_bf16_bits(
                        w2[(size_t)(32 * nt + (lane & 31)) * dff + 32 * t + 16 * s + 8 * (j >> 2) + 4 * (lane >> 5) + (j & 3)]);
}
unsigned char cn_f32_to_e4m3_host(float f) {
    const unsigned char sign = std::signbit(f) ? 0x80 : 0;
    float a = std::fabs(f);
    if (a != a) return 0x7f;
    if (a >= 448.f) return sign | 0x7e;
    if (a < 0.0009765625f) return sign;
    int e;
    (void)std::frexp(a, &e);
    int E = e - 1;
    if (E < -6) {
        const int r = (int)std::nearbyint(a * 512.f);
        return sign | (unsigned char)(r >= 8 ? 0x08 : r);
    }
    int r = (int)std::nearbyint((a / std::ldexp(1.f, E) - 1.f) * 8.f);
    if (r == 8) {
        r = 0;
        ++E;
    }
    const int bits = ((E + 7) << 3) | r;
    return sign | (unsigned char)(bits > 0x7e ? 0x7e : bits);
}
int cn_e4m3_exp(float mx) { return mx > 0.f ? (int)std::floor(std::log2(448.f / mx)) : 0; }

static void ch_pack_w1_f8(const float* w1, int p, float scale, unsigned char* out) {
    for (int t = 0; t < 8; ++t)
        for (int lane = 0; lane < 64; ++lane)
            for (int e = 0; e < 32; ++e) {
                const int s = t >> 2, kk = t & 3, r = e & 15;
                const int k = 64 * kk + 32 * (e >> 4) + 8 * (r >> 2) + 4 * (lane >> 5) + (r & 3);
                out[((size_t)(2 * t + (e >> 4)) * 64 + lane) * 16 + r] =
                    cn_f32_to_e4m3_host(w1[(size_t)(64 * p + 32 * s + (lane & 31)) * CH_D + k] * scale);
            }
}
static void ch_pack_w2_f8(const float* w2, int dff, int p, float scale, unsigned char* out) {
    for (int nt = 0; nt < 8; ++nt)
        for (int lane = 0; lane < 64; ++lane)
            for (int e = 0; e < 32; ++e) {
                const int r = e & 15;
                const int k = 64 * p + 32 * (e >> 4) + 8 * (r >> 2) + 4 * (lane >> 5) + (r & 3);
                out[((size_t)(2 * nt + (e >> 4)) * 64 + lane) * 16 + r] =
                    cn_f32_to_e4m3_host(w2[(size_t)(32 * nt + (lane & 31)) * dff + k] * scale);
            }
}
static float ch_f8_scale(const float* w, size_t n) {
    float mx = 0.f;
    for (size_t i = 0; i < n; ++i) mx = std::max(mx, std::fabs(w[i]));
    return std::ldexp(1.f, cn_e4m3_exp(mx));
}

void pack_chain(const ChainWeights& w, uint16_t* stream, float* tab, int* f8_q) {
    const size_t unit = CH_UNIT_BYTES / 2;
    size_t u = 0;
    const bool f8 = f8_q != nullptr;
    if (w.wo)
        for (int rt = 0; rt < 8; ++rt) ch_pack_rows(w.wo, CH_D, rt, false, stream + unit * u++);
    const int nt_ffn = f8 ? w.dff / 64 : w.dff / 32;
    float ln_mul = 1.f, hid_mul = 1.f;
    if (f8 && nt_ffn > 0) {
        const float s1 = ch_f8_scale(w.w1, (size_t)w.dff * CH_D), s2 = ch_f8_scale(w.w2, (size_t)w.dff * CH_D);
        ln_mul = CHAIN_F8_S_LN;
        hid_mul = CHAIN_F8_S_HID;
        f8_q[0] = 127 - (int)std::lround(std::log2(s1));
        f8_q[1] = 127 + (int)std::lround(std::log2(hid_mul)) - (int)std::lround(std::log2(ln_mul));
        f8_q[2] = 127 - (int)std::lround(std::log2(s2));
        f8_q[3] = 127 - (int)std::lround(std::log2(hid_mul));
        unsigned char* bytes = reinterpret_cast<unsigned char*>(stream);
        ch_pack_w1_f8(w.w1, 0, s1, bytes + CH_UNIT_BYTES * u++);
        for (int p = 0; p + 1 < nt_ffn; ++p) {
            ch_pack_w1_f8(w.w1, p + 1, s1, bytes + CH_UNIT_BYTES * u++);
            ch_pack_w2_f8(w.w2, w.dff, p, s2, bytes + CH_UNIT_BYTES * u++);
        }
        ch_pack_w2_f8(w.w2, w.dff, nt_ffn - 1, s2, bytes + CH_UNIT_BYTES * u++);
    } else {
        if (nt_ffn > 0) ch_pack_rows(w.w1, CH_D, 0, true, stream + unit * u++);
        for (int t = 0; t + 1 < nt_ffn; ++t) {
            ch_pack_rows(w.w1, CH_D, t + 1, true, stream + unit * u++);
            ch_pack_w2(w.w2, w.dff, t, stream + unit * u++);
        }
        if (nt_ffn > 0) ch_pack_w2(w.w2, w.dff, nt_ffn - 1, stream + unit * u++);
    }
    for (int jt = 0; jt < w.tail_n / 32; ++jt) ch_pack_rows(w.wt, CH_D, jt, true, stream + unit * u++);
    memset(tab, 0, sizeof(float) * CH_TAB_FLOATS);
    auto put = [&](int off, const float* src, int n, float mul) {
        if (src)
            for (int i = 0; i < n; ++i) tab[off + i] = src[i] * mul;
    };
    put(CT_BO, w.bo, CH_D, 1.f);
    put(CT_LN1A, w.ln1_a, CH_D, ln_mul);
    put(CT_LN1B, w.ln1_b, CH_D, ln_mul);
    put(CT_B2, w.b2, CH_D, 1.f);
    put(CT_NLNA, w.nln_a, CH_D, 1.f);
    put(CT_NLNB, w.nln_b, CH_D, 1.f);
    put(CT_BT, w.bt, w.tail_n, 1.f);
    put(CT_B1, w.b1, w.dff, hid_mul);
}
```

### cassnat_asr_public_amd/csrc/ops.hip

```cpp
#include <algorithm>
#include <cmath>
#include <cstring>
#include <string>
#include <thread>
#include <vector>

#include "../../include/cassnat_hip.h"
#include "kernels.h"

namespace {

class Scratch {
  public:
    Scratch(const char* who, hipStream_t s) : who_(who), s_(s) {}
    Scratch(const Scratch&) = delete;
    Scratch& operator=(const Scratch&) = delete;
    ~Scratch() {
        (void)hipStreamSynchronize(s_);
        for (void* p : bufs_) (void)hipFree(p);
    }
    bool ok() const { return ok_; }
    void* alloc(size_t bytes) {
        if (!ok_) return nullptr;
        void* p = nullptr;
        const hipError_t e = hipMalloc(&p, bytes);
        if (e != hipSuccess) return fail("hipMalloc", bytes, e);
        bufs_.push_back(p);
        return p;
    }
    void* upload(const void* host, size_t bytes) {
        void* p = alloc(bytes);
        if (!p) return nullptr;
        const hipError_t e = hipMemcpy(p, host, bytes, hipMemcpyHostToDevice);
        return e == hipSuccess ? p : fail("hipMemcpy", bytes, e);
    }
    int finish(int rc) {
        const hipError_t e = hipStreamSynchronize(s_);
        if (rc == 0 && e != hipSuccess) {
            cn_set_error(std::string(who_) + ": " + hipGetErrorString(e));
            return -2;
        }
        return rc;
    }

  private:
    void* fail(const char* what, size_t bytes, hipError_t e) {
        cn_set_error(std::string(who_) + ": " + what + " of " + std::to_string(bytes) + " bytes failed: " + hipGetErrorString(e));
        ok_ = false;
        return nullptr;
    }
    const char* who_;
    hipStream_t s_;
    std::vector<void*> bufs_;
    bool ok_ = true;
};

std::vector<unsigned char> split_rows256(const float* x, int M) {
    std::vector<unsigned char> hx((size_t)M * 1024);
    for (size_t r = 0; r < (size_t)M; ++r)
        for (size_t c = 0; c < 256; ++c) {
            const float v = x[r * 256 + c];
            const uint16_t hi = cn_host_op16(v);
            const uint32_t hbits = (uint32_t)hi << 16;
            float hf;
            std::memcpy(&hf, &hbits, 4);
            const uint16_t lo = cn_host_op16(v - hf);
            std::memcpy(&hx[r * 1024 + cn_split_off(c)], &hi, 2);
            std::memcpy(&hx[r * 1024 + cn_split_off(c) + 64], &lo, 2);
        }
    return hx;
}

}

static FbankOpts fbank_opts_from(const cn_fbank_opts* o) {
    FbankOpts f;
    f.sample_rate = o->sample_rate;
    f.frame_length_ms = o->frame_length_ms;
    f.frame_shift_ms = o->frame_shift_ms;
    f.preemph = o->preemph;
    f.low_freq = o->low_freq;
    f.high_freq = o->high_freq;
    f.num_mel = o->num_mel;
    f.window_type = o->window_type;
    f.remove_dc = o->remove_dc;
    f.use_power = o->use_power;
    f.use_log = o->use_log;
    return f;
}

extern "C" void cn_fbank_default_opts(cn_fbank_opts* o) {
    if (!o) return;
    const FbankOpts f;
    std::memset(o, 0, sizeof(*o));
    o->sample_rate = f.sample_rate;
    o->frame_length_ms = f.frame_length_ms;
    o->frame_shift_ms = f.frame_shift_ms;
    o->preemph = f.preemph;
    o->low_freq = f.low_freq;
    o->high_freq = f.high_freq;
    o->num_mel = f.num_mel;
    o->window_type = f.window_type;
    o->remove_dc = f.remove_dc;
    o->use_power = f.use_power;
    o->use_log = f.use_log;
}

extern "C" int32_t cn_fbank_num_frames(const cn_fbank_opts* o, int32_t num_samples) {
    return o ? fbank_num_frames(fbank_opts_from(o), num_samples) : 0;
}

extern "C" int cn_fbank(const cn_fbank_opts* o, const float* wave_dev, const int32_t* num_samples_dev, int32_t B,
                        int32_t max_samples, const float* cmvn_mean_dev, const float* cmvn_istd_dev, float* feats_dev,
                        int32_t Tmax, float pad_value, void* stream) {
    if (!o || !wave_dev || !num_samples_dev || !feats_dev || B < 0 || max_samples < 0 || Tmax < 0) {
        cn_set_error("cn_fbank: bad argument");
        return -1;
    }
    return launch_fbank(fbank_opts_from(o), wave_dev, num_samples_dev, B, max_samples, cmvn_mean_dev, cmvn_istd_dev, feats_dev,
                        Tmax, pad_value, (hipStream_t)stream);
}

extern "C" int cn_op_gemm(int32_t precision, const void* A, int32_t lda, const void* W, const float* bias, void* C,
                          int32_t ldc, int32_t c_is_f32, int32_t M, int32_t N, int32_t K, int32_t relu,
                          const float* resid, int32_t ldr, const float* pe, int32_t pe_period, float scale,
                          void* stream) {
    if ((precision = cn_own_precision(precision, "cn_op_gemm")) < 0) return -1;
    GemmArgs g;
    g.A = A;
    g.lda = lda;
    g.W = W;
    g.bias = bias;
    g.C = C;
    g.ldc = ldc;
    g.c_f32 = c_is_f32;
    g.M = M;
    g.N = N;
    g.K = K;
    g.epi = (relu ? CN_EPI_RELU : 0) | (resid ? CN_EPI_RESID : 0) | (pe ? CN_EPI_EMBED : 0);
    g.resid = resid;
    g.ldr = ldr;
    g.pe = pe;
    g.pe_period = pe_period;
    g.scale = scale;
    return launch_gemm(precision, g, (hipStream_t)stream);
}

extern "C" int cn_op_convert(int32_t precision, const void* src, void* dst, int64_t n, int32_t to_f32, void* stream) {
    if ((precision = cn_own_precision(precision, "cn_op_convert")) < 0) return -1;
    if (n < 0 || !src || !dst) {
        cn_set_error("cn_op_convert: bad argument");
        return -1;
    }
    return to_f32 ? launch_convert_back(precision, src, (float*)dst, (size_t)n, (hipStream_t)stream)
                  : launch_convert(precision, (const float*)src, dst, (size_t)n, (hipStream_t)stream);
}

extern "C" int cn_op_conv1(int32_t precision, const float* x, const float* w9c, const float* bias, void* out, int32_t B,
                           int32_t T, int32_t F, int32_t C, void* stream) {
    if ((precision = cn_own_precision(precision, "cn_op_conv1")) < 0) return -1;
    return launch_conv1(precision, x, w9c, bias, out, B, T, F, (T - 1) / 2 + 1, (F - 1) / 2 + 1, C, 0, (hipStream_t)stream);
}

extern "C" int cn_op_conv1_bordered(const float* x, const float* w9c, const float* bias, void* out, int32_t B, int32_t T, int32_t F,
                                    int32_t C, void* stream) {
    return launch_conv1_bordered_bf16(x, w9c, bias, out, B, T, F, (T - 1) / 2 + 1, (F - 1) / 2 + 1, C, (hipStream_t)stream);
}

extern "C" int cn_op_conv_frontend_fp8(const float* x_dev, const float* w1_9c_dev, const float* b1_dev, const float* w2_host,
                                       const float* b2_dev, void* out_dev, void* img8_out_dev, int32_t B, int32_t T, int32_t F,
                                       int32_t C, float img_scale, float out8_scale, float* w_scale_out, void* stream) {
    if (!conv2_f8_applies(C, C)) {
        cn_set_error("cn_op_conv_frontend_fp8: 256 channels only");
        return -1;
    }
    hipStream_t s = (hipStream_t)stream;
    const int T1 = (T - 1) / 2 + 1, F1 = (F - 1) / 2 + 1, T2 = (T1 - 1) / 2 + 1, F2 = (F1 - 1) / 2 + 1;
    std::vector<unsigned char> w8((size_t)C * 9 * C);
    const int lg = pack_conv2_f8(w2_host, C, 9 * C, C, 1, w8.data());
    if (w_scale_out) *w_scale_out = std::ldexp(1.f, lg);
    const int q[4] = {127 - lg, 127 - (int)std::lround(std::log2(img_scale)), 0, 0};
    const size_t img_bytes = (size_t)B * (T1 + 2) * (F1 + 2) * C;
    Scratch sc("cn_op_conv_frontend_fp8", s);
    void* dw = sc.upload(w8.data(), w8.size());
    void* dq = sc.upload(q, 16);
    void* img = sc.alloc(img_bytes);
    if (!sc.ok()) return -2;
    CN_HIP_CHECK(hipMemsetAsync(img, 0xff, img_bytes, s));
    int rc = launch_conv1_f8(x_dev, w1_9c_dev, b1_dev, img, B, T, F, T1, F1, C, 1, img_scale, s);
    if (rc == 0) rc = launch_conv2_f8(img, dw, (const int*)dq, b2_dev, out_dev, B, T1, F1, T2, F2, s, out8_scale);
    if (rc == 0 && img8_out_dev) CN_HIP_CHECK(hipMemcpyAsync(img8_out_dev, img, img_bytes, hipMemcpyDeviceToDevice, s));
    return sc.finish(rc);
}

extern "C" int cn_op_conv_frontend_mix(const float* x_dev, const float* w1_9c_dev, const float* b1_dev, const float* w2_host,
                                       const float* b2_dev, void* out_dev, void* img_out_dev, int32_t B, int32_t T, int32_t F, int32_t C,
                                       void* stream) {
    if (!conv2_mix_applies(CN_PREC_X3, C, C)) {
        cn_set_error("cn_op_conv_frontend_mix: 256 channels only (and not in the half-precision build of the library)");
        return -1;
    }
    hipStream_t s = (hipStream_t)stream;
    const int T1 = (T - 1) / 2 + 1, F1 = (F - 1) / 2 + 1, T2 = (T1 - 1) / 2 + 1, F2 = (F1 - 1) / 2 + 1;
    const size_t n = (size_t)C * 9 * C;
    std::vector<unsigned char> w(4 * n);
    int q[4];
    pack_conv2_mix(w2_host, C, 9 * C, C, 1, w.data(), q);
    const size_t img_bytes = (size_t)B * (T1 + 2) * (F1 + 2) * C * 4;
    Scratch sc("cn_op_conv_frontend_mix", s);
    void* dw = sc.upload(w.data(), w.size());
    void* dq = sc.upload(q, 16);
    void* img = sc.alloc(img_bytes);
    if (!sc.ok()) return -2;
    CN_HIP_CHECK(hipMemsetAsync(img, 0xff, img_bytes, s));
    int rc = launch_conv1_mixplanes(x_dev, w1_9c_dev, b1_dev, img, B, T, F, T1, F1, C, 1, std::ldexp(1.f, MIX_LG_AL), std::ldexp(1.f, MIX_LG_AQ), s);
    if (rc == 0)
        rc = launch_conv2_mix(img, dw, (const unsigned char*)dw + 2 * n, (const unsigned char*)dw + 3 * n, (const int*)dq, b2_dev, out_dev, B, T1, F1,
                              T2, F2, s);
    if (rc == 0 && img_out_dev) CN_HIP_CHECK(hipMemcpyAsync(img_out_dev, img, img_bytes, hipMemcpyDeviceToDevice, s));
    return sc.finish(rc);
}

extern "C" int cn_op_linear256_fp8(const void* a8_dev, const float* w_host, const float* bias_dev, float* out_dev, int32_t M, int32_t K,
                                   float a_scale, float out_scale, const float* pe_dev, int32_t pe_period, float* w_scale_out,
                                   void* stream) {
    if (!linear256_f8_applies(256, K)) {
        cn_set_error("cn_op_linear256_fp8: K must be 5120");
        return -1;
    }
    hipStream_t s = (hipStream_t)stream;
    float mx = 0.f;
    for (size_t i = 0; i < (size_t)256 * K; ++i) mx = std::max(mx, std::fabs(w_host[i]));
    const int lg = cn_e4m3_exp(mx);
    const float ws = std::ldexp(1.f, lg);
    if (w_scale_out) *w_scale_out = ws;
    std::vector<unsigned char> w8((size_t)256 * K);
    for (size_t i = 0; i < w8.size(); ++i) w8[i] = cn_f32_to_e4m3_host(w_host[i] * ws);
    const int q[4] = {127 - lg, 127 - (int)std::lround(std::log2(a_scale)), 0, 0};
    Scratch sc("cn_op_linear256_fp8", s);
    void* dw = sc.upload(w8.data(), w8.size());
    void* dq = sc.upload(q, 16);
    if (!sc.ok()) return -2;
    return sc.finish(launch_linear256_f8(a8_dev, dw, (const int*)dq, bias_dev, out_dev, M, K, out_scale, pe_dev, pe_period, s));
}

extern "C" int cn_op_conv2(int32_t precision, const void* conv1_out, const void* w_khwc, const float* bias, void* out,
                           int32_t B, int32_t T1, int32_t F1, int32_t C, void* stream) {
    if ((precision = cn_own_precision(precision, "cn_op_conv2")) < 0) return -1;
    GemmArgs g;
    const int T2 = (T1 - 1) / 2 + 1, F2 = (F1 - 1) / 2 + 1;
    g.A = conv1_out;
    g.W = w_khwc;
    g.bias = bias;
    g.C = out;
    g.ldc = C;
    g.M = B * T2 * F2;
    g.N = C;
    g.K = 9 * C;
    g.epi = CN_EPI_RELU;
    g.conv = 1;
    g.cB = B;
    g.cT1 = T1;
    g.cF1 = F1;
    g.cC = C;
    g.cT2 = T2;
    g.cF2 = F2;
    if (!conv2_dma_applies(precision, C, C)) return launch_gemm(precision, g, (hipStream_t)stream);
    const size_t cell = (size_t)C * 2, prow = (size_t)(F1 + 2) * cell;
    Scratch sc("cn_op_conv2", (hipStream_t)stream);
    void* padded = sc.alloc((size_t)B * (T1 + 2) * prow);
    if (!sc.ok()) return -2;
    CN_HIP_CHECK(hipMemsetAsync(padded, 0, (size_t)B * (T1 + 2) * prow, (hipStream_t)stream));
    for (int b = 0; b < B; ++b)
        CN_HIP_CHECK(hipMemcpy2DAsync((unsigned char*)padded + ((size_t)b * (T1 + 2) + 1) * prow + cell, prow,
                                      (const unsigned char*)conv1_out + (size_t)b * T1 * F1 * cell, (size_t)F1 * cell,
                                      (size_t)F1 * cell, T1, hipMemcpyDeviceToDevice, (hipStream_t)stream));
    g.A = padded;
    g.conv_halo = 1;
    return sc.finish(launch_gemm(precision, g, (hipStream_t)stream));
}

extern "C" int cn_op_layernorm(int32_t precision, const float* x, const float* a2, const float* b2, void* y, int32_t M,
                               int32_t d, float eps, void* stream) {
    if ((precision = cn_own_precision(precision, "cn_op_layernorm")) < 0) return -1;
    return launch_layernorm(precision, x, a2, b2, y, 0, M, d, eps, (hipStream_t)stream);
}

extern "C" int cn_op_attention(int32_t precision, const void* Q, int32_t ldq, const void* K, int32_t ldk, const void* V,
                               int32_t ldv, void* O, int32_t ldo, int32_t B, int32_t H, int32_t Lq, int32_t Lk,
                               const uint8_t* keymask, const int32_t* klen, const int32_t* intervals, int32_t iv_stride,
                               int32_t causal, float scale, void* stream) {
    if ((precision = cn_own_precision(precision, "cn_op_attention")) < 0) return -1;
    AttnArgs a;
    a.Q = Q;
    a.K = K;
    a.V = V;
    a.O = O;
    a.ldq = ldq;
    a.ldk = ldk;
    a.ldv = ldv;
    a.ldo = ldo;
    a.B = B;
    a.H = H;
    a.Lq = Lq;
    a.Lk = Lk;
    a.keymask = keymask;
    a.klen = klen;
    a.intervals = intervals;
    a.iv_stride = iv_stride;
    a.causal = causal;
    a.scale = scale;
    int rc = launch_attention(precision, a, (hipStream_t)stream);
    if (rc == 0 && cn_exp_env("CASSNAT_ATTN_STAMPS")) {
        (void)hipStreamSynchronize((hipStream_t)stream);
        (void)attention_print_stamps();
    }
    return rc;
}

extern "C" int cn_op_attention_desc(int32_t precision, const cn_attn_desc* d, void* stream) {
    if ((precision = cn_own_precision(precision, "cn_op_attention_desc")) < 0) return -1;
    if (!d) {
        cn_set_error("cn_op_attention_desc: null descriptor");
        return -1;
    }
    AttnArgs a;
    a.Q = d->Q;
    a.K = d->K;
    a.V = d->V;
    a.O = d->O;
    a.ldq = d->ldq;
    a.ldk = d->ldk;
    a.ldv = d->ldv;
    a.ldo = d->ldo;
    a.B = d->B;
    a.H = d->H;
    a.Lq = d->Lq;
    a.Lk = d->Lk;
    a.keymask = d->keymask;
    a.kv_mod = d->kv_mod;
    a.kv_index = d->kv_index;
    a.klen = d->klen;
    a.kcap = d->kcap;
    a.kcap_stride = d->kcap_stride;
    a.q_blocked = d->q_blocked;
    a.kv_blocked = d->kv_blocked;
    a.q_col = d->q_col;
    a.k_col = d->k_col;
    a.v_col = d->v_col;
    a.q_n = d->q_n;
    a.kv_n = d->kv_n;
    a.o_blocked = d->o_blocked;
    a.intervals = d->intervals;
    a.iv_stride = d->iv_stride;
    a.causal = d->causal;
    a.scale = d->scale;
    a.rel_pos = d->rel_pos;
    a.rel_u = d->rel_u;
    a.rel_v = d->rel_v;
    a.rel_R = d->rel_R;
    a.ld_pos = d->ld_pos;
    return launch_attention(precision, a, (hipStream_t)stream);
}

extern "C" int32_t cn_attn_desc_size(void) { return (int32_t)sizeof(cn_attn_desc); }

extern "C" int cn_op_logsoftmax_argmax(float* logits, int32_t M, int32_t V, int32_t* arg, float* maxlp,
                                       int32_t write_logp, void* stream) {
    return launch_logsoftmax_argmax(logits, M, V, V, arg, maxlp, write_logp, (hipStream_t)stream);
}

extern "C" int cn_op_ctc_align(const int32_t* best, const uint8_t* keymask, const float* size_ratio, int32_t B,
                               int32_t Tp, int32_t blank, int32_t left, int32_t right, int32_t* shift,
                               int32_t* src_size, int32_t* ylen, int32_t* ymax, int32_t* intervals, void* stream) {
    AlignArgs a;
    a.best = best;
    a.keymask = keymask;
    a.size_ratio = size_ratio;
    a.B = B;
    a.Tp = Tp;
    a.blank = blank;
    a.left = left;
    a.right = right;
    a.shift = shift;
    a.src_size = src_size;
    a.ylen = ylen;
    a.ymax = ymax;
    a.intervals = intervals;
    return launch_ctc_align(a, (hipStream_t)stream);
}

extern "C" int cn_op_ctc_prefix_beam(const float* logp, const float* size_ratio, int32_t B, int32_t Tp, int32_t V, int32_t beam,
                                     int32_t pruning, double length_penalty, int32_t blank, int32_t* hyp, int32_t hyp_cap,
                                     int32_t* hyp_len, double* score, double* p_blk, double* p_nblk, int32_t* nbeam, void* stream) {
    hipStream_t s = (hipStream_t)stream;
    const size_t M = (size_t)B * Tp;
    const int P = pruning > 0 ? pruning : 1;
    Scratch sc("cn_op_ctc_prefix_beam", s);
    int* top_idx = (int*)sc.alloc(M * P * 4);
    float* top_val = (float*)sc.alloc(M * P * 4);
    unsigned char* hpar = (unsigned char*)sc.alloc(M * (size_t)std::max(beam, 1));
    int* htok = (int*)sc.alloc(M * (size_t)std::max(beam, 1) * 4);
    if (!sc.ok()) return -2;
    int rc = pruning > 0 ? launch_topk(logp, (int)M, V, V, pruning, top_idx, top_val, s) : 0;
    if (rc == 0) {
        CtcBeamArgs a;
        a.logp = logp;
        a.top_idx = top_idx;
        a.size_ratio = size_ratio;
        a.B = B;
        a.Tp = Tp;
        a.V = V;
        a.P = pruning;
        a.W = beam;
        a.blank = blank;
        a.Lmax = hyp_cap;
        a.lp = length_penalty;
        a.hist_parent = hpar;
        a.hist_tok = htok;
        a.hyp = hyp;
        a.hyp_len = hyp_len;
        a.score = score;
        a.p_blk = p_blk;
        a.p_nblk = p_nblk;
        a.n_out = nbeam;
        rc = launch_ctc_prefix_beam(a, s);
    }
    return sc.finish(rc);
}

extern "C" int cn_op_ctc_viterbi(const float* logp, const uint8_t* keymask, const float* size_ratio, const int32_t* labels,
                                 const int32_t* label_len, int32_t B, int32_t Tp, int32_t V, int32_t ld, int32_t ymax, int32_t blank,
                                 int32_t* out_path, void* stream) {
    hipStream_t s = (hipStream_t)stream;
    Scratch sc("cn_op_ctc_viterbi", s);
    unsigned char* bp = (unsigned char*)sc.alloc((size_t)B * Tp * (2 * (size_t)ymax + 1));
    if (!sc.ok()) return -2;
    ViterbiArgs v;
    v.logp = logp;
    v.keymask = keymask;
    v.size_ratio = size_ratio;
    v.labels = labels;
    v.label_len = label_len;
    v.B = B;
    v.Tp = Tp;
    v.V = V;
    v.ld = ld;
    v.ymax = ymax;
    v.blank = blank;
    v.bp = bp;
    v.out_path = out_path;
    return sc.finish(launch_ctc_viterbi(v, s));
}

extern "C" int cn_op_greedy_pack(const int32_t* tok, const float* val, const int32_t* ylen, int32_t B, int32_t U,
                                 int32_t sos, int32_t hyp_stride, int32_t* hyp, int32_t* hyp_len, double* score,
                                 void* stream) {
    return launch_greedy_pack(tok, val, ylen, B, U, sos, hyp_stride, hyp, hyp_len, score, (hipStream_t)stream);
}

extern "C" int cn_op_topk(const float* logp, int32_t M, int32_t V, int32_t k, int32_t* idx, float* val, void* stream) {
    return launch_topk(logp, M, V, V, k, idx, val, (hipStream_t)stream);
}

extern "C" int cn_op_gemm_fp8(const void* a_bf16_dev, int32_t lda, const float* w_host, const float* bias_dev, float* c_dev,
                              int32_t M, int32_t N, int32_t K, float a_scale, int32_t relu, float* w_scale_out, void* stream) {
    if (M < 1 || N < 1 || K < 128 || K % 128 != 0) {
        cn_set_error("cn_op_gemm_fp8: K must be a positive multiple of 128");
        return -1;
    }
    hipStream_t s = (hipStream_t)stream;
    float mx = 0.f;
    for (size_t i = 0; i < (size_t)N * K; ++i) mx = std::max(mx, std::fabs(w_host[i]));
    const float ws = std::ldexp(1.f, cn_e4m3_exp(mx));
    if (w_scale_out) *w_scale_out = ws;
    std::vector<unsigned char> w8((size_t)N * K);
    for (size_t i = 0; i < w8.size(); ++i) w8[i] = cn_f32_to_e4m3_host(w_host[i] * ws);
    Scratch sc("cn_op_gemm_fp8", s);
    void* dw = sc.upload(w8.data(), w8.size());
    void* da = sc.alloc((size_t)M * K);
    if (!sc.ok()) return -2;
    int rc = launch_quantize_fp8(a_bf16_dev, lda, da, M, K, a_scale, s);
    if (rc == 0) {
        GemmArgs g;
        g.A = da;
        g.lda = K;
        g.W = dw;
        g.bias = bias_dev;
        g.C = c_dev;
        g.ldc = N;
        g.c_f32 = 1;
        g.M = M;
        g.N = N;
        g.K = K;
        g.epi = relu ? CN_EPI_RELU : 0;
        g.ab_fp8 = 1;
        g.acc_scale = 1.f / (a_scale * ws);
        rc = launch_gemm(CN_PREC_BF16, g, s);
    }
    return sc.finish(rc);
}

extern "C" int cn_op_cmvn(float* feats_dev, const int32_t* len_dev, const double* mean_dev, const double* std_dev, int32_t B, int32_t T,
                          int32_t F, void* stream) {
    if (!feats_dev || !len_dev || !mean_dev || !std_dev) {
        cn_set_error("cn_op_cmvn: null argument");
        return -1;
    }
    return launch_cmvn(feats_dev, len_dev, mean_dev, std_dev, B, T, F, (hipStream_t)stream);
}

extern "C" int cn_host_gather(void* dst, const uint64_t* src_ptrs, const uint64_t* dst_offsets, const uint64_t* nbytes, int32_t n,
                              int32_t threads) {
    if (!dst || !src_ptrs || !dst_offsets || !nbytes || n < 0) {
        cn_set_error("cn_host_gather: null argument");
        return -1;
    }
    auto run = [&](int lo, int hi) {
        for (int i = lo; i < hi; ++i)
            memcpy(static_cast<unsigned char*>(dst) + dst_offsets[i], reinterpret_cast<const void*>(src_ptrs[i]), nbytes[i]);
    };
    const int nt = std::max(1, std::min<int>(threads, n));
    if (nt == 1) {
        run(0, n);
        return 0;
    }
    uint64_t total = 0;
    for (int i = 0; i < n; ++i) total += nbytes[i];
    std::vector<std::thread> pool;
    int lo = 0;
    uint64_t acc = 0;
    for (int t = 0; t < nt; ++t) {
        int hi = lo;
        const uint64_t want = total * (uint64_t)(t + 1) / (uint64_t)nt;
        while (hi < n && (t + 1 == nt || acc + nbytes[hi] <= want || hi == lo)) acc += nbytes[hi++];
        if (t + 1 < nt) pool.emplace_back(run, lo, hi);
        else run(lo, hi);
        lo = hi;
    }
    for (auto& th : pool) th.join();
    return 0;
}

extern "C" int cn_op_unpack_rows(const float* packed_dev, const int32_t* off_dev, const int32_t* len_dev, float* out_dev, int32_t rows,
                                 int32_t T, int32_t F, float pad, const double* mean_dev, const double* std_dev, void* stream) {
    if (!packed_dev || !off_dev || !len_dev || !out_dev || (!mean_dev) != (!std_dev)) {
        cn_set_error("cn_op_unpack_rows: null argument (mean and std come together)");
        return -1;
    }
    return launch_unpack_rows(packed_dev, off_dev, len_dev, out_dev, rows, T, F, pad, mean_dev, std_dev, (hipStream_t)stream);
}

extern "C" int cn_op_quantize_fp8(const void* src_bf16_dev, int32_t ld, void* dst_dev, int32_t M, int32_t K, float scale,
                                  void* stream) {
    return launch_quantize_fp8(src_bf16_dev, ld, dst_dev, M, K, scale, (hipStream_t)stream);
}

extern "C" int cn_op_logsoftmax_topk(const float* logits, int32_t M, int32_t V, float temperature, int32_t k, int32_t* idx,
                                     float* val, void* stream) {
    return launch_logsoftmax_topk(logits, M, V, V, temperature, k, idx, val, (hipStream_t)stream);
}

extern "C" int cn_op_logsoftmax_fuse_topk(const float* att, const float* lm, int32_t M, int32_t V, float temperature, float w,
                                          int32_t k, int32_t* idx, float* val, void* stream) {
    if (M < 0 || V < 1 || (M > 0 && (!att || !lm || !idx || !val))) {
        cn_set_error("cn_op_logsoftmax_fuse_topk: bad argument");
        return -1;
    }
    return launch_logsoftmax_fuse_topk(att, lm, M, V, V, temperature, w, k, idx, val, (hipStream_t)stream);
}

extern "C" int cn_op_logsoftmax_gather(const float* logits, int32_t M, int32_t V, const int32_t* cand, int32_t k, float* out,
                                       void* stream) {
    if (M < 0 || V < 1 || (M > 0 && (!logits || !cand || !out))) {
        cn_set_error("cn_op_logsoftmax_gather: bad argument");
        return -1;
    }
    return launch_logsoftmax_gather(logits, M, V, V, cand, k, out, (hipStream_t)stream);
}

extern "C" int cn_op_ast_gather_attn(int32_t precision, int32_t mode, const void* q, int32_t ldq, void* k, void* v, void* o,
                                     int32_t ldo, int32_t n, int32_t H, int32_t nkeys, int32_t slots, int32_t d, int32_t table_stride,
                                     const int32_t* anc, const uint8_t* keyok, const int32_t* utt, const uint8_t* keymask, float scale,
                                     int32_t append_pos, void* stream) {
    if ((precision = cn_own_precision(precision, "cn_op_ast_gather_attn")) < 0) return -1;
    if (precision != CN_PREC_F32 && precision != CN_PREC_BF16 && precision != CN_PREC_X3) {
        cn_set_error("cn_op_ast_gather_attn: precision must be F32, BF16 (F16 in the half-precision build) or BF16X3");
        return -1;
    }
    if (mode != 0 && mode != 1) {
        cn_set_error("cn_op_ast_gather_attn: mode must be 0 (cache) or 1 (source memory)");
        return -1;
    }
    if (n < 0 || H < 1 || H > 16 || d != 64 * H || nkeys < 1 || ldo < d || ldq < (mode == 0 ? 3 * d : d) || !q || !k || !v ||
        (n > 0 && !o)) {
        cn_set_error("cn_op_ast_gather_attn: need 1 <= H <= 16, d = 64 * H, nkeys >= 1, ldo >= d and ldq >= 3d (mode 0) / d (mode 1)");
        return -1;
    }
    if (mode == 0 && (slots < n || table_stride < nkeys || append_pos < -1 || append_pos >= nkeys || !anc || !keyok)) {
        cn_set_error("cn_op_ast_gather_attn: mode 0 needs slots >= n, table_stride >= nkeys, -1 <= append_pos < nkeys, anc and keyok");
        return -1;
    }
    if (mode == 1 && (!utt || !keymask)) {
        cn_set_error("cn_op_ast_gather_attn: mode 1 needs utt and keymask");
        return -1;
    }
    GatherAttnArgs a;
    a.q = q;
    a.ldq = ldq;
    a.k = k;
    a.v = v;
    a.o = o;
    a.ldo = ldo;
    a.n = n;
    a.H = H;
    a.nkeys = nkeys;
    a.slots = slots;
    a.d = d;
    a.table_stride = table_stride;
    a.anc = anc;
    a.keyok = keyok;
    a.utt = utt;
    a.keymask = keymask;
    a.scale = scale;
    a.append_pos = mode == 0 ? append_pos : -1;
    return launch_ast_gather_attn(precision, mode, a, (hipStream_t)stream);
}

extern "C" int cn_op_ast_ctc_prepare(float* logp, const uint8_t* keymask, float* r0, int32_t B, int32_t Tp, int32_t V, int32_t blank,
                                     void* stream) {
    if (B < 1 || Tp < 1 || V < 1 || blank < 0 || blank >= V || !logp || !keymask || !r0) {
        cn_set_error("cn_op_ast_ctc_prepare: need B, Tp, V >= 1, 0 <= blank < V and non-null buffers");
        return -1;
    }
    return launch_ast_ctc_prepare(logp, keymask, r0, B, Tp, V, blank, (hipStream_t)stream);
}

extern "C" int cn_op_ast_ctc_prefix(const float* logp, const float* r0, const float* r_prev, float* r_new, const int32_t* utt,
                                    const int32_t* last_tok, const int32_t* cand, const int32_t* prev_ref, float* score, int32_t n,
                                    int32_t K, int32_t Tp, int32_t V, int32_t blank, int32_t eos, int32_t out_len, void* stream) {
    if (n < 0 || K < 1 || Tp < 1 || V < 1 || blank < 0 || blank >= V || out_len < 0 || out_len > Tp ||
        (n > 0 && (!logp || !r0 || !r_new || !utt || !last_tok || !cand || !prev_ref || !score))) {
        cn_set_error("cn_op_ast_ctc_prefix: need n >= 0, K, Tp, V >= 1, 0 <= blank < V, 0 <= out_len <= Tp and non-null buffers");
        return -1;
    }
    CtcPrefixArgs a;
    a.logp = logp;
    a.r0 = r0;
    a.r_prev = r_prev;
    a.r_new = r_new;
    a.utt = utt;
    a.last_tok = last_tok;
    a.cand = cand;
    a.prev_ref = prev_ref;
    a.score = score;
    a.n = n;
    a.K = K;
    a.Tp = Tp;
    a.V = V;
    a.blank = blank;
    a.eos = eos;
    a.out_len = out_len;
    return launch_ast_ctc_prefix(a, (hipStream_t)stream);
}

static int ast_beam_state_of(AstBeamState& st, int32_t* tok0, int32_t* tok1, int32_t* anc0, int32_t* anc1, uint8_t* keyok0,
                             uint8_t* keyok1, int32_t* len0, int32_t* len1, double* score0, double* score1, int32_t* valid0,
                             int32_t* valid1, int32_t* ctc_ref0, int32_t* ctc_ref1, float* ctc_prev0, float* ctc_prev1, int32_t* cur_tok,
                             int32_t* utt, int32_t* live, const char* who) {
    const void* all[] = {tok0, tok1, anc0, anc1, keyok0, keyok1, len0, len1, score0, score1, valid0, valid1, ctc_ref0, ctc_ref1,
                         ctc_prev0, ctc_prev1, cur_tok, utt, live};
    for (const void* ptr : all)
        if (!ptr) {
            cn_set_error(std::string(who) + ": null state array");
            return -1;
        }
    st.tok[0] = tok0;
    st.tok[1] = tok1;
    st.anc[0] = anc0;
    st.anc[1] = anc1;
    st.keyok[0] = keyok0;
    st.keyok[1] = keyok1;
    st.len[0] = len0;
    st.len[1] = len1;
    st.score[0] = score0;
    st.score[1] = score1;
    st.valid[0] = valid0;
    st.valid[1] = valid1;
    st.ctc_ref[0] = ctc_ref0;
    st.ctc_ref[1] = ctc_ref1;
    st.ctc_prev[0] = ctc_prev0;
    st.ctc_prev[1] = ctc_prev1;
    st.cur_tok = cur_tok;
    st.utt = utt;
    st.live = live;
    return 0;
}

extern "C" int cn_op_ast_beam_init(int32_t* tok0, int32_t* tok1, int32_t* anc0, int32_t* anc1, uint8_t* keyok0, uint8_t* keyok1,
                                   int32_t* len0, int32_t* len1, double* score0, double* score1, int32_t* valid0, int32_t* valid1,
                                   int32_t* ctc_ref0, int32_t* ctc_ref1, float* ctc_prev0, float* ctc_prev1, int32_t* cur_tok, int32_t* utt,
                                   int32_t* live, int32_t cur, int32_t B, int32_t bw, int32_t L, int32_t sos, int32_t pad, void* stream) {
    if (B < 1 || bw < 1 || bw > 32 || L < 1 || (cur != 0 && cur != 1)) {
        cn_set_error("cn_op_ast_beam_init: need B >= 1, 1 <= beam_width <= 32, L >= 1 and cur 0 or 1");
        return -1;
    }
    AstBeamState st;
    CN_TRY(ast_beam_state_of(st, tok0, tok1, anc0, anc1, keyok0, keyok1, len0, len1, score0, score1, valid0, valid1, ctc_ref0, ctc_ref1,
                             ctc_prev0, ctc_prev1, cur_tok, utt, live, "cn_op_ast_beam_init"));
    return launch_ast_beam_init(st, cur, B, bw, L, sos, pad, (hipStream_t)stream);
}

extern "C" int cn_op_ast_beam_update(int32_t* tok0, int32_t* tok1, int32_t* anc0, int32_t* anc1, uint8_t* keyok0, uint8_t* keyok1,
                                     int32_t* len0, int32_t* len1, double* score0, double* score1, int32_t* valid0, int32_t* valid1,
                                     int32_t* ctc_ref0, int32_t* ctc_ref1, float* ctc_prev0, float* ctc_prev1, int32_t* cur_tok,
                                     int32_t* utt, int32_t* live, const int32_t* idx, const float* att, const float* ctc, const float* lm,
                                     int32_t cur, int32_t pos, int32_t bw, int32_t K, int32_t L, int32_t eos, int32_t sos, int32_t pad,
                                     int32_t use_ctc, int32_t use_lp, int32_t use_lm, float w, float u, float lw, double lp, int32_t B,
                                     void* stream) {
    if (B < 1 || bw < 1 || bw > 32 || K < bw || K > 32 || L < 1 || (cur != 0 && cur != 1) || !idx || !att || (use_ctc && !ctc) ||
        (use_ctc && use_lm && !lm)) {
        cn_set_error("cn_op_ast_beam_update: need B >= 1, 1 <= beam_width <= K <= 32, L >= 1, cur 0 or 1 and the step's arrays");
        return -1;
    }
    AstBeamState st;
    CN_TRY(ast_beam_state_of(st, tok0, tok1, anc0, anc1, keyok0, keyok1, len0, len1, score0, score1, valid0, valid1, ctc_ref0, ctc_ref1,
                             ctc_prev0, ctc_prev1, cur_tok, utt, live, "cn_op_ast_beam_update"));
    AstBeamStep q;
    q.idx = idx;
    q.att = att;
    q.ctc = ctc;
    q.lm = lm;
    q.cur = cur;
    q.pos = pos;
    q.bw = bw;
    q.K = K;
    q.L = L;
    q.eos = eos;
    q.sos = sos;
    q.pad = pad;
    q.use_ctc = use_ctc;
    q.use_lp = use_lp;
    q.use_lm = use_lm;
    q.w = w;
    q.u = u;
    q.lw = lw;
    q.lp = lp;
    return launch_ast_beam_update(st, q, B, (hipStream_t)stream);
}

extern "C" int cn_op_nat_lm_fuse_topk(const float* att, const float* lm, const int32_t* last, const int32_t* zlen, int32_t B, int32_t U,
                                      int32_t V, int32_t bw, int32_t step, float w, int32_t k, int32_t* idx, float* val, void* stream) {
    if (B < 1 || V < 1 || !att || !lm || !idx || !val) {
        cn_set_error("cn_op_nat_lm_fuse_topk: bad argument");
        return -1;
    }
    NatFuseArgs a;
    a.att = att;
    a.lm = lm;
    a.last = last;
    a.zlen = zlen;
    a.idx = idx;
    a.val = val;
    a.U = U;
    a.V = V;
    a.bw = bw;
    a.step = step;
    a.k = k;
    a.w = w;
    return launch_nat_lm_fuse_topk(a, B * bw, (hipStream_t)stream);
}

extern "C" int cn_op_nat_beam_update(int32_t* tok0, int32_t* tok1, int32_t* anc0, int32_t* anc1, uint8_t* keyok0, uint8_t* keyok1,
                                     double* score0, double* score1, int32_t* cur_tok, const int32_t* idx, const float* val,
                                     const int32_t* last, int32_t cur, int32_t step, int32_t bw, int32_t L, int32_t pad, int32_t use_lp,
                                     double lp, int32_t B, void* stream) {
    const void* all[] = {tok0, tok1, anc0, anc1, keyok0, keyok1, score0, score1, cur_tok, idx, val, last};
    for (const void* ptr : all)
        if (!ptr) {
            cn_set_error("cn_op_nat_beam_update: null array");
            return -1;
        }
    NatBeamState st;
    st.tok[0] = tok0;
    st.tok[1] = tok1;
    st.anc[0] = anc0;
    st.anc[1] = anc1;
    st.keyok[0] = keyok0;
    st.keyok[1] = keyok1;
    st.score[0] = score0;
    st.score[1] = score1;
    st.cur_tok = cur_tok;
    NatBeamStep q;
    q.idx = idx;
    q.val = val;
    q.last = last;
    q.cur = cur;
    q.step = step;
    q.bw = bw;
    q.L = L;
    q.pad = pad;
    q.use_lp = use_lp;
    q.lp = lp;
    return launch_nat_beam_update(st, q, B, (hipStream_t)stream);
}

extern "C" int cn_op_ctc_lm_frame(double* pb, double* pnb, double* sctc, double* slm, int32_t* len, int32_t* last, int32_t* nb, int32_t* tok,
                                  int32_t* pos, int32_t* parent, int32_t* stay, const int32_t* rowid_cur, int32_t* rowid_nxt,
                                  uint8_t* hist_parent, int32_t* hist_tok, const float* logp, const int32_t* top_idx, const float* lmrow,
                                  const int32_t* frames, const int32_t* count, int32_t B, int32_t Tp, int32_t V, int32_t W, int32_t P,
                                  int32_t blank, int32_t sos, int32_t iter, int32_t Lt, int32_t hist_stride, double lp, double lm_weight,
                                  void* stream) {
    const void* all[] = {pb, pnb, sctc, slm, len, last, nb, tok, pos, parent, stay, rowid_cur, rowid_nxt, hist_parent, hist_tok, logp,
                         top_idx, lmrow, frames, count};
    for (const void* ptr : all)
        if (!ptr) {
            cn_set_error("cn_op_ctc_lm_frame: null array");
            return -1;
        }
    if (B < 1 || V < 1 || sos < 0 || sos >= V) {
        cn_set_error("cn_op_ctc_lm_frame: need B >= 1 and sos inside the vocabulary");
        return -1;
    }
    CtcLmState st;
    st.pb = pb;
    st.pnb = pnb;
    st.sctc = sctc;
    st.slm = slm;
    st.len = len;
    st.last = last;
    st.nb = nb;
    st.tok = tok;
    st.pos = pos;
    st.parent = parent;
    st.stay = stay;
    st.rowid[iter & 1] = const_cast<int32_t*>(rowid_cur);
    st.rowid[(iter & 1) ^ 1] = rowid_nxt;
    CtcLmFrame a;
    a.logp = logp;
    a.top_idx = top_idx;
    a.lmrow = lmrow;
    a.frames = frames;
    a.count = count;
    a.hist_parent = hist_parent;
    a.hist_tok = hist_tok;
    a.B = B;
    a.Tp = Tp;
    a.V = V;
    a.P = P;
    a.W = W;
    a.blank = blank;
    a.sos = sos;
    a.iter = iter;
    a.Lt = Lt;
    a.hist_stride = hist_stride;
    a.lp = lp;
    a.lm_weight = lm_weight;
    return launch_ctc_lm_frame(st, a, (hipStream_t)stream);
}

extern "C" int cn_op_ctc_lm_rows(const float* fresh, const float* prv, float* nxt, const int32_t* parent, const int32_t* stay,
                                 const int32_t* count, int32_t iter, int32_t slots, int32_t W, int32_t V, void* stream) {
    if (!fresh || !prv || !nxt || !parent || !stay) {
        cn_set_error("cn_op_ctc_lm_rows: null array");
        return -1;
    }
    return launch_ctc_lm_rows(fresh, prv, nxt, parent, stay, count, iter, slots, W, V, (hipStream_t)stream);
}

extern "C" int cn_op_ffn_fused(float* x_dev, const float* ln_a_dev, const float* ln_b_dev, const float* w1_host,
                               const float* b1_dev, const float* w2_host, const float* b2_dev, const float* nln_a_dev,
                               const float* nln_b_dev, void* xn_out_dev, int32_t M, int32_t dff, float eps,
                               int32_t nslice, void* stream) {
    return cn_op_ffn_fused_act(x_dev, ln_a_dev, ln_b_dev, w1_host, b1_dev, w2_host, b2_dev, nln_a_dev, nln_b_dev, xn_out_dev, M, dff, eps,
                               nslice, CN_ACT_RELU, stream);
}

extern "C" int cn_op_ffn_fused_act(float* x_dev, const float* ln_a_dev, const float* ln_b_dev, const float* w1_host,
                                   const float* b1_dev, const float* w2_host, const float* b2_dev, const float* nln_a_dev,
                                   const float* nln_b_dev, void* xn_out_dev, int32_t M, int32_t dff, float eps,
                                   int32_t nslice, int32_t act, void* stream) {
    if (act != CN_ACT_RELU && act != CN_ACT_SWISH) {
        cn_set_error("cn_op_ffn_fused_act: act must be CN_ACT_RELU or CN_ACT_SWISH");
        return -1;
    }
    if (dff <= 0 || dff % 128 != 0 || dff > 2048) {
        cn_set_error("cn_op_ffn_fused: d_ff must be a positive multiple of 128, at most 2048");
        return -1;
    }
    const size_t n = (size_t)dff * 256;
    std::vector<uint16_t> h1(n), h2(n);
    pack_ffn_w1(w1_host, dff, h1.data());
    pack_ffn_w2(w2_host, dff, h2.data());
    Scratch sc("cn_op_ffn_fused", (hipStream_t)stream);
    FfnFusedArgs a;
    a.x = x_dev;
    a.ln_a = ln_a_dev;
    a.ln_b = ln_b_dev;
    a.w1p = sc.upload(h1.data(), n * 2);
    a.b1 = b1_dev;
    a.w2p = sc.upload(h2.data(), n * 2);
    a.b2 = b2_dev;
    a.nln_a = nln_a_dev;
    a.nln_b = nln_b_dev;
    a.xn_out = xn_out_dev;
    a.M = M;
    a.d = 256;
    a.dff = dff;
    a.eps = eps;
    a.act = act == CN_ACT_SWISH ? FF_ACT_SWISH : FF_ACT_RELU;
    if (nslice > 1) {
        a.nslice = nslice;
        a.partial = (float*)sc.alloc((size_t)nslice * M * 256 * 4);
    }
    if (!sc.ok()) return -2;
    int rc = launch_ffn_fused(a, (hipStream_t)stream);
    if (rc == 0 && nslice > 1)
        rc = launch_ffn_reduce(x_dev, a.partial, nslice, b2_dev, nln_a_dev, nln_b_dev, xn_out_dev, M, eps, (hipStream_t)stream);
    return sc.finish(rc);
}

extern "C" int cn_op_ffn_x3(float* x_dev, const float* ln_a_dev, const float* ln_b_dev, const float* w1_host, const float* b1_dev,
                            const float* w2_host, const float* b2_dev, const float* nln_a_dev, const float* nln_b_dev,
                            void* xn_out_dev, int32_t M, int32_t dff, float eps, int32_t mix, void* stream) {
    return cn_op_ffn_x3_act(x_dev, ln_a_dev, ln_b_dev, w1_host, b1_dev, w2_host, b2_dev, nln_a_dev, nln_b_dev, xn_out_dev, M, dff, eps, mix,
                            CN_ACT_RELU, stream);
}

extern "C" int cn_op_ffn_x3_act(float* x_dev, const float* ln_a_dev, const float* ln_b_dev, const float* w1_host, const float* b1_dev,
                                const float* w2_host, const float* b2_dev, const float* nln_a_dev, const float* nln_b_dev,
                                void* xn_out_dev, int32_t M, int32_t dff, float eps, int32_t mix, int32_t act, void* stream) {
    if (act != CN_ACT_RELU && (act != CN_ACT_SWISH || mix)) {
        cn_set_error("cn_op_ffn_x3_act: act must be CN_ACT_RELU, or CN_ACT_SWISH without the mixed arithmetic");
        return -1;
    }
    if (!ffn_x3_applies(256, dff)) {
        cn_set_error("cn_op_ffn_x3: d_ff must be a positive multiple of 128, at most 2048");
        return -1;
    }
    const size_t bytes = ffn_x3_stream_bytes(dff);
    std::vector<uint16_t> h(bytes / 2);
    pack_ffn_x3(w1_host, w2_host, dff, h.data(), mix != 0);
    Scratch sc("cn_op_ffn_x3", (hipStream_t)stream);
    FfnX3Args a;
    a.x = x_dev;
    a.ln_a = ln_a_dev;
    a.ln_b = ln_b_dev;
    a.wst = sc.upload(h.data(), bytes);
    a.mix = mix != 0;
    a.b1 = b1_dev;
    a.b2 = b2_dev;
    a.nln_a = nln_a_dev;
    a.nln_b = nln_b_dev;
    a.xn_out = xn_out_dev;
    a.M = M;
    a.d = 256;
    a.dff = dff;
    a.eps = eps;
    a.act = act == CN_ACT_SWISH ? FF_ACT_SWISH : FF_ACT_RELU;
    if (!sc.ok()) return -2;
    return sc.finish(launch_ffn_x3(a, (hipStream_t)stream));
}

extern "C" int cn_op_x3_chain(float* x_dev, const void* ctx_dev, const float* wo_host, const float* bo_dev, const float* ln_a_dev,
                              const float* ln_b_dev, const float* w1_host, const float* b1_dev, const float* w2_host,
                              const float* b2_dev, const float* nln_a_dev, const float* nln_b_dev, void* xn_out_dev,
                              const float* wt_host, const float* bt_dev, void* tail_out_dev, int32_t tail_n, int32_t M, int32_t dff,
                              float eps, int32_t mix, void* stream) {
    if (!ffn_x3_applies(256, dff) || (wt_host && !proj_x3_applies(tail_n, 256))) {
        cn_set_error("cn_op_x3_chain: d_ff a multiple of 128 (<= 2048), tail_n a multiple of 32 (<= 1024)");
        return -1;
    }
    Scratch sc("cn_op_x3_chain", (hipStream_t)stream);
    FfnX3Args a;
    {
        std::vector<uint16_t> h(ffn_x3_stream_bytes(dff) / 2);
        pack_ffn_x3(w1_host, w2_host, dff, h.data(), mix != 0);
        a.wst = sc.upload(h.data(), h.size() * 2);
        a.mix = mix != 0;
    }
    if (ctx_dev) {
        std::vector<unsigned char> h((size_t)256 * 1024);
        pack_proj_x3(wo_host, 256, h.data());
        a.ctx = ctx_dev;
        a.wo_p = sc.upload(h.data(), h.size());
        a.bo = bo_dev;
    }
    if (wt_host) {
        std::vector<unsigned char> h((size_t)tail_n * 1024);
        pack_proj_x3(wt_host, tail_n, h.data());
        a.tail_p = sc.upload(h.data(), h.size());
        a.tail_b = bt_dev;
        a.tail_out = tail_out_dev;
        a.tail_n = tail_n;
        a.ld_tail = tail_n;
    }
    a.x = x_dev;
    a.ln_a = ln_a_dev;
    a.ln_b = ln_b_dev;
    a.b1 = b1_dev;
    a.b2 = b2_dev;
    a.nln_a = nln_a_dev;
    a.nln_b = nln_b_dev;
    a.xn_out = xn_out_dev;
    a.M = M;
    a.d = 256;
    a.dff = dff;
    a.eps = eps;
    if (!sc.ok()) return -2;
    return sc.finish(launch_ffn_x3(a, (hipStream_t)stream));
}

extern "C" int cn_op_chain(float* x_dev, const void* ctx_dev, int32_t ldctx, const float* wo_host, const float* bo_host,
                           const float* ln1_a_host, const float* ln1_b_host, const float* w1_host, const float* b1_host,
                           const float* w2_host, const float* b2_host, const float* nln_a_host, const float* nln_b_host,
                           const float* wt_host, const float* bt_host, void* out_dev, int32_t ldo, int32_t M, int32_t dff,
                           int32_t tail_n, float eps, int32_t x_mode, void* stream) {
    if (dff < 0 || dff % 32 != 0 || dff > 2048 || tail_n < 0 || tail_n % 32 != 0 || tail_n > 1536) {
        cn_set_error("cn_op_chain: d_ff and the tail width must be multiples of 32 (<= 2048 / <= 1536)");
        return -1;
    }
    ChainWeights w;
    w.wo = ctx_dev ? wo_host : nullptr;
    w.bo = bo_host;
    w.ln1_a = ln1_a_host;
    w.ln1_b = ln1_b_host;
    w.w1 = w1_host;
    w.b1 = b1_host;
    w.w2 = w2_host;
    w.b2 = b2_host;
    w.nln_a = nln_a_host;
    w.nln_b = nln_b_host;
    w.wt = wt_host;
    w.bt = bt_host;
    w.dff = dff;
    w.tail_n = tail_n;
    const int f8 = (x_mode & 32) != 0;
    if (f8 && (dff <= 0 || dff % 256 != 0 || (x_mode & 8))) {
        cn_set_error("cn_op_chain: the e4m3 feed-forward form (x_mode bit 32) needs d_ff % 256 == 0 and the ReLU activation");
        return -1;
    }
    const size_t units = chain_stream_units(ctx_dev != nullptr, dff, tail_n, f8);
    std::vector<uint16_t> hs((units + 7) * (CHAIN_UNIT_BYTES / 2));
    std::vector<float> ht(CHAIN_TAB_FLOATS + 4);
    int hq[4] = {127, 127, 127, 127};
    pack_chain(w, hs.data(), ht.data(), f8 ? hq : nullptr);
    std::memcpy(&ht[CHAIN_TAB_FLOATS], hq, 16);
    Scratch sc("cn_op_chain", (hipStream_t)stream);
    void* ds = sc.upload(hs.data(), hs.size() * 2);
    const float* dt = (const float*)sc.upload(ht.data(), ht.size() * 4);
    if (!sc.ok()) return -2;
    ChainArgs a;
    a.x = x_dev;
    a.ctx = ctx_dev;
    a.ldctx = ldctx;
    a.wstream = ds;
    a.tab = dt;
    a.out = out_dev;
    a.ldo = ldo;
    a.M = M;
    a.d = 256;
    a.dff = dff;
    a.tail_n = tail_n;
    a.has_next = nln_a_host != nullptr;
    a.eps = eps;
    a.x_in_blocked = (x_mode & 1) != 0;
    a.x_out_blocked = (x_mode & 2) != 0;
    a.store_x = (x_mode & 4) == 0;
    a.swish = (x_mode & 8) != 0;
    a.out_blocked = (x_mode & 16) != 0;
    a.f8 = f8;
    a.f8_q = f8 ? reinterpret_cast<const int*>(dt + CHAIN_TAB_FLOATS) : nullptr;
    int rc = launch_chain(a, (hipStream_t)stream);
    if (const char* rep = cn_exp_env("CASSNAT_CHAIN_REPEAT")) {
        const int ns = cn_exp_env("CASSNAT_CHAIN_STREAMS") ? atoi(cn_exp_env("CASSNAT_CHAIN_STREAMS")) : 0;
        std::vector<hipStream_t> ss(ns > 0 ? ns : 0);
        for (auto& q : ss) (void)hipStreamCreateWithFlags(&q, hipStreamNonBlocking);
        (void)hipStreamSynchronize((hipStream_t)stream);
        for (int i = 1; i < atoi(rep) && rc == 0; ++i) rc = launch_chain(a, ns > 0 ? ss[i % ns] : (hipStream_t)stream);
        for (auto& q : ss) {
            (void)hipStreamSynchronize(q);
            (void)hipStreamDestroy(q);
        }
    }
    rc = sc.finish(rc);
    if (cn_exp_env("CASSNAT_CHAIN_STAMPS")) (void)chain_print_stamps();
    return rc;
}

static int op_genmax_impl(const void* h_dev, const float* w_host, const float* b_host, int32_t M, int32_t V,
                          int32_t* arg_dev, float* maxlp_dev, const int32_t* tgt_dev, float* tgt_lp_dev, int32_t U, int32_t ld,
                          void* stream) {
    const int vtw = genmax_vtw(V);
    if (vtw > 48) {
        cn_set_error("cn_op_genmax: V too large");
        return -1;
    }
    std::vector<uint16_t> hw((size_t)4 * vtw * 16 * 512);
    std::vector<float> hb((size_t)4 * vtw * 32);
    pack_genmax(w_host, b_host, V, hw.data(), hb.data());
    Scratch sc("cn_op_genmax", (hipStream_t)stream);
    GenmaxArgs a;
    a.h = h_dev;
    a.wp = sc.upload(hw.data(), hw.size() * 2);
    a.bp = (const float*)sc.upload(hb.data(), hb.size() * 4);
    if (!sc.ok()) return -2;
    a.arg = arg_dev;
    a.maxlp = maxlp_dev;
    a.M = M;
    a.V = V;
    a.d = 256;
    a.tgt = tgt_dev;
    a.tgt_lp = tgt_lp_dev;
    a.tgt_U = U;
    a.tgt_ld = ld;
    int rc = launch_genmax(a, (hipStream_t)stream);
    if (const char* rep = cn_exp_env("CASSNAT_GENMAX_REPEAT"))
        for (int i = 1, n = atoi(rep); rc == 0 && i < n; ++i) rc = launch_genmax(a, (hipStream_t)stream);
    return sc.finish(rc);
}

extern "C" int cn_op_genmax(const void* h_dev, const float* w_host, const float* b_host, int32_t M, int32_t V,
                            int32_t* arg_dev, float* maxlp_dev, void* stream) {
    return op_genmax_impl(h_dev, w_host, b_host, M, V, arg_dev, maxlp_dev, nullptr, nullptr, 0, 0, stream);
}

extern "C" int cn_op_genmax_gather(const void* h_dev, const float* w_host, const float* b_host, int32_t B, int32_t U, int32_t V,
                                   const int32_t* tgt_dev, int32_t ld, float* tgt_lp_dev, void* stream) {
    return op_genmax_impl(h_dev, w_host, b_host, B * U, V, nullptr, nullptr, tgt_dev, tgt_lp_dev, U, ld, stream);
}

extern "C" int cn_op_genmax_x3(const float* h_host, const float* w_host, const float* b_host, int32_t M, int32_t V, int32_t* arg_dev,
                               float* maxlp_dev, const int32_t* tgt_dev, int32_t U, int32_t ld, float* tgt_lp_dev, void* stream) {
    if (!genmax_applies(CN_PREC_X3, 256, V) || M < 1) {
        cn_set_error("cn_op_genmax_x3: V too large");
        return -1;
    }
    const int vtw = genmax_x3_vtw(V);
    std::vector<uint16_t> hw((size_t)8 * vtw * 16 * 1024);
    std::vector<float> hb((size_t)8 * vtw * 32);
    pack_genmax_x3(w_host, b_host, V, hw.data(), hb.data());
    const std::vector<unsigned char> hx = split_rows256(h_host, M);
    Scratch sc("cn_op_genmax_x3", (hipStream_t)stream);
    GenmaxArgs a;
    a.x3 = true;
    a.h = sc.upload(hx.data(), hx.size());
    a.wp = sc.upload(hw.data(), hw.size() * 2);
    a.bp = (const float*)sc.upload(hb.data(), hb.size() * 4);
    if (!sc.ok()) return -2;
    a.arg = arg_dev;
    a.maxlp = maxlp_dev;
    a.M = M;
    a.V = V;
    a.d = 256;
    a.tgt = tgt_dev;
    a.tgt_lp = tgt_lp_dev;
    a.tgt_U = U;
    a.tgt_ld = ld;
    int rc = launch_genmax(a, (hipStream_t)stream);
    if (const char* rep = cn_exp_env("CASSNAT_GENMAX_REPEAT"))
        for (int i = 1, n = atoi(rep); rc == 0 && i < n; ++i) rc = launch_genmax(a, (hipStream_t)stream);
    return sc.finish(rc);
}

extern "C" int cn_op_proj_x3(const float* a_host, const float* w_host, const float* bias_host, const float* resid_dev,
                             float resid_scale, void* c_dev, int32_t M, int32_t N, int32_t split_out, void* stream) {
    if (!proj_x3_applies(N, 256) || M < 1) {
        cn_set_error("cn_op_proj_x3: N must be a multiple of 32, at most 1024");
        return -1;
    }
    std::vector<unsigned char> hw((size_t)N * 1024);
    pack_proj_x3(w_host, N, hw.data());
    const std::vector<unsigned char> hx = split_rows256(a_host, M);
    Scratch sc("cn_op_proj_x3", (hipStream_t)stream);
    ProjX3Args a;
    a.A = sc.upload(hx.data(), hx.size());
    a.lda = 256;
    a.wp = sc.upload(hw.data(), hw.size());
    a.bias = (const float*)sc.upload(bias_host, (size_t)N * 4);
    if (!sc.ok()) return -2;
    a.C = c_dev;
    a.ldc = N;
    a.c_f32 = split_out ? 0 : 1;
    a.resid = resid_dev;
    a.ldr = N;
    a.resid_scale = resid_scale;
    a.M = M;
    a.N = N;
    return sc.finish(launch_proj_x3(a, (hipStream_t)stream));
}
```

Before: 50060 utt/s.

## Fuse chain prologue loads with first out-projection stage to overlap x/ctx/weight fetch

Replaces the separate prologue (table DMA, ring prefill, x/ctx row loads with a full vmcnt(0) wait and barrier) with a single asm prologue. It loads x directly into the accumulator registers and interleaves the ctx, table and ring-unit LDS DMAs with the first out-projection MFMA stage, using graded vmcnt waits. The goal is to hide global-load latency at the kernel start instead of stalling on all loads. It also adds a blocked-ctx mode flag in the host op and a stamp for prologue+S1. The hand-scheduled vmcnt counts and fixed AGPR assignments are fragile and could be wrong for some layouts.

Measured after the change: 50330 utt/s, median of 6. No clear change (+0.5%).

```diff
diff --git a/cassnat_asr_public_amd/csrc/chain.hip b/cassnat_asr_public_amd/csrc/chain.hip
--- a/cassnat_asr_public_amd/csrc/chain.hip
+++ b/cassnat_asr_public_amd/csrc/chain.hip
@@ -175,103 +175,6 @@
     }
 }
 
-template <int XS, int CS, bool CTX>
-__device__ __forceinline__ void ch_load_rows(f32x4 (&xr)[32], bf16x8 (&bop)[16], const float* const (&xb)[8], const bf16* const (&cb)[4]) {
-    if constexpr (CTX) {
-        asm volatile("global_load_dwordx4 %[x0], %[xb0], off\n\t"
-                     "global_load_dwordx4 %[x1], %[xb0], off offset:%[xo1]\n\t"
-                     "global_load_dwordx4 %[x2], %[xb0], off offset:%[xo2]\n\t"
-                     "global_load_dwordx4 %[x3], %[xb0], off offset:%[xo3]\n\t"
-                     "global_load_dwordx4 %[x4], %[xb1], off\n\t"
-                     "global_load_dwordx4 %[x5], %[xb1], off offset:%[xo1]\n\t"
-                     "global_load_dwordx4 %[x6], %[xb1], off offset:%[xo2]\n\t"
-                     "global_load_dwordx4 %[x7], %[xb1], off offset:%[xo3]\n\t"
-                     "global_load_dwordx4 %[x8], %[xb2], off\n\t"
-                     "global_load_dwordx4 %[x9], %[xb2], off offset:%[xo1]\n\t"
-                     "global_load_dwordx4 %[x10], %[xb2], off offset:%[xo2]\n\t"
-                     "global_load_dwordx4 %[x11], %[xb2], off offset:%[xo3]\n\t"
-                     "global_load_dwordx4 %[x12], %[xb3], off\n\t"
-                     "global_load_dwordx4 %[x13], %[xb3], off offset:%[xo1]\n\t"
-                     "global_load_dwordx4 %[x14], %[xb3], off offset:%[xo2]\n\t"
-                     "global_load_dwordx4 %[x15], %[xb3], off offset:%[xo3]\n\t"
-                     "global_load_dwordx4 %[x16], %[xb4], off\n\t"
-                     "global_load_dwordx4 %[x17], %[xb4], off offset:%[xo1]\n\t"
-                     "global_load_dwordx4 %[x18], %[xb4], off offset:%[xo2]\n\t"
-                     "global_load_dwordx4 %[x19], %[xb4], off offset:%[xo3]\n\t"
-                     "global_load_dwordx4 %[x20], %[xb5], off\n\t"
-                     "global_load_dwordx4 %[x21], %[xb5], off offset:%[xo1]\n\t"
-                     "global_load_dwordx4 %[x22], %[xb5], off offset:%[xo2]\n\t"
-                     "global_load_dwordx4 %[x23], %[xb5], off offset:%[xo3]\n\t"
-                     "global_load_dwordx4 %[x24], %[xb6], off\n\t"
-                     "global_load_dwordx4 %[x25], %[xb6], off offset:%[xo1]\n\t"
-                     "global_load_dwordx4 %[x26], %[xb6], off offset:%[xo2]\n\t"
-                     "global_load_dwordx4 %[x27], %[xb6], off offset:%[xo3]\n\t"
-                     "global_load_dwordx4 %[x28], %[xb7], off\n\t"
-                     "global_load_dwordx4 %[x29], %[xb7], off offset:%[xo1]\n\t"
-                     "global_load_dwordx4 %[x30], %[xb7], off offset:%[xo2]\n\t"
-                     "global_load_dwordx4 %[x31], %[xb7], off offset:%[xo3]\n\t"
-                     "global_load_dwordx4 %[c0], %[cb0], off\n\t"
-                     "global_load_dwordx4 %[c1], %[cb0], off offset:%[co1]\n\t"
-                     "global_load_dwordx4 %[c2], %[cb0], off offset:%[co2]\n\t"
-                     "global_load_dwordx4 %[c3], %[cb0], off offset:%[co3]\n\t"
-                     "global_load_dwordx4 %[c4], %[cb1], off\n\t"
-                     "global_load_dwordx4 %[c5], %[cb1], off offset:%[co1]\n\t"
-                     "global_load_dwordx4 %[c6], %[cb1], off offset:%[co2]\n\t"
-                     "global_load_dwordx4 %[c7], %[cb1], off offset:%[co3]\n\t"
-                     "global_load_dwordx4 %[c8], %[cb2], off\n\t"
-                     "global_load_dwordx4 %[c9], %[cb2], off offset:%[co1]\n\t"
-                     "global_load_dwordx4 %[c10], %[cb2], off offset:%[co2]\n\t"
-                     "global_load_dwordx4 %[c11], %[cb2], off offset:%[co3]\n\t"
-                     "global_load_dwordx4 %[c12], %[cb3], off\n\t"
-                     "global_load_dwordx4 %[c13], %[cb3], off offset:%[co1]\n\t"
-                     "global_load_dwordx4 %[c14], %[cb3], off offset:%[co2]\n\t"
-                     "global_load_dwordx4 %[c15], %[cb3], off offset:%[co3]\n\t"
-                     "s_waitcnt vmcnt(0)"
-                     : [x0] "=&a"(xr[0]), [x1] "=&a"(xr[1]), [x2] "=&a"(xr[2]), [x3] "=&a"(xr[3]), [x4] "=&a"(xr[4]), [x5] "=&a"(xr[5]), [x6] "=&a"(xr[6]), [x7] "=&a"(xr[7]), [x8] "=&a"(xr[8]), [x9] "=&a"(xr[9]), [x10] "=&a"(xr[10]), [x11] "=&a"(xr[11]), [x12] "=&a"(xr[12]), [x13] "=&a"(xr[13]), [x14] "=&a"(xr[14]), [x15] "=&a"(xr[15]), [x16] "=&a"(xr[16]), [x17] "=&a"(xr[17]), [x18] "=&a"(xr[18]), [x19] "=&a"(xr[19]), [x20] "=&a"(xr[20]), [x21] "=&a"(xr[21]), [x22] "=&a"(xr[22]), [x23] "=&a"(xr[23]), [x24] "=&a"(xr[24]), [x25] "=&a"(xr[25]), [x26] "=&a"(xr[26]), [x27] "=&a"(xr[27]), [x28] "=&a"(xr[28]), [x29] "=&a"(xr[29]), [x30] "=&a"(xr[30]), [x31] "=&a"(xr[31]), [c0] "=&v"(bop[0]), [c1] "=&v"(bop[1]), [c2] "=&v"(bop[2]), [c3] "=&v"(bop[3]), [c4] "=&v"(bop[4]), [c5] "=&v"(bop[5]), [c6] "=&v"(bop[6]), [c7] "=&v"(bop[7]), [c8] "=&v"(bop[8]), [c9] "=&v"(bop[9]), [c10] "=&v"(bop[10]), [c11] "=&v"(bop[11]), [c12] "=&v"(bop[12]), [c13] "=&v"(bop[13]), [c14] "=&v"(bop[14]), [c15] "=&v"(bop[15])
-                     : [xb0] "v"(xb[0]), [xb1] "v"(xb[1]), [xb2] "v"(xb[2]), [xb3] "v"(xb[3]), [xb4] "v"(xb[4]), [xb5] "v"(xb[5]), [xb6] "v"(xb[6]), [xb7] "v"(xb[7]), [cb0] "v"(cb[0]), [cb1] "v"(cb[1]), [cb2] "v"(cb[2]), [cb3] "v"(cb[3])
-                       , [xo1] "n"(XS), [xo2] "n"(2 * XS), [xo3] "n"(3 * XS), [co1] "n"(CS), [co2] "n"(2 * CS), [co3] "n"(3 * CS)
-                     : "memory");
-    } else {
-        asm volatile("global_load_dwordx4 %[x0], %[xb0], off\n\t"
-                     "global_load_dwordx4 %[x1], %[xb0], off offset:%[xo1]\n\t"
-                     "global_load_dwordx4 %[x2], %[xb0], off offset:%[xo2]\n\t"
-                     "global_load_dwordx4 %[x3], %[xb0], off offset:%[xo3]\n\t"
-                     "global_load_dwordx4 %[x4], %[xb1], off\n\t"
-                     "global_load_dwordx4 %[x5], %[xb1], off offset:%[xo1]\n\t"
-                     "global_load_dwordx4 %[x6], %[xb1], off offset:%[xo2]\n\t"
-                     "global_load_dwordx4 %[x7], %[xb1], off offset:%[xo3]\n\t"
-                     "global_load_dwordx4 %[x8], %[xb2], off\n\t"
-                     "global_load_dwordx4 %[x9], %[xb2], off offset:%[xo1]\n\t"
-                     "global_load_dwordx4 %[x10], %[xb2], off offset:%[xo2]\n\t"
-                     "global_load_dwordx4 %[x11], %[xb2], off offset:%[xo3]\n\t"
-                     "global_load_dwordx4 %[x12], %[xb3], off\n\t"
-                     "global_load_dwordx4 %[x13], %[xb3], off offset:%[xo1]\n\t"
-                     "global_load_dwordx4 %[x14], %[xb3], off offset:%[xo2]\n\t"
-                     "global_load_dwordx4 %[x15], %[xb3], off offset:%[xo3]\n\t"
-                     "global_load_dwordx4 %[x16], %[xb4], off\n\t"
-                     "global_load_dwordx4 %[x17], %[xb4], off offset:%[xo1]\n\t"
-                     "global_load_dwordx4 %[x18], %[xb4], off offset:%[xo2]\n\t"
-                     "global_load_dwordx4 %[x19], %[xb4], off offset:%[xo3]\n\t"
-                     "global_load_dwordx4 %[x20], %[xb5], off\n\t"
-                     "global_load_dwordx4 %[x21], %[xb5], off offset:%[xo1]\n\t"
-                     "global_load_dwordx4 %[x22], %[xb5], off offset:%[xo2]\n\t"
-                     "global_load_dwordx4 %[x23], %[xb5], off offset:%[xo3]\n\t"
-                     "global_load_dwordx4 %[x24], %[xb6], off\n\t"
-                     "global_load_dwordx4 %[x25], %[xb6], off offset:%[xo1]\n\t"
-                     "global_load_dwordx4 %[x26], %[xb6], off offset:%[xo2]\n\t"
-                     "global_load_dwordx4 %[x27], %[xb6], off offset:%[xo3]\n\t"
-                     "global_load_dwordx4 %[x28], %[xb7], off\n\t"
-                     "global_load_dwordx4 %[x29], %[xb7], off offset:%[xo1]\n\t"
-                     "global_load_dwordx4 %[x30], %[xb7], off offset:%[xo2]\n\t"
-                     "global_load_dwordx4 %[x31], %[xb7], off offset:%[xo3]\n\t"
-                     "s_waitcnt vmcnt(0)"
-                     : [x0] "=&a"(xr[0]), [x1] "=&a"(xr[1]), [x2] "=&a"(xr[2]), [x3] "=&a"(xr[3]), [x4] "=&a"(xr[4]), [x5] "=&a"(xr[5]), [x6] "=&a"(xr[6]), [x7] "=&a"(xr[7]), [x8] "=&a"(xr[8]), [x9] "=&a"(xr[9]), [x10] "=&a"(xr[10]), [x11] "=&a"(xr[11]), [x12] "=&a"(xr[12]), [x13] "=&a"(xr[13]), [x14] "=&a"(xr[14]), [x15] "=&a"(xr[15]), [x16] "=&a"(xr[16]), [x17] "=&a"(xr[17]), [x18] "=&a"(xr[18]), [x19] "=&a"(xr[19]), [x20] "=&a"(xr[20]), [x21] "=&a"(xr[21]), [x22] "=&a"(xr[22]), [x23] "=&a"(xr[23]), [x24] "=&a"(xr[24]), [x25] "=&a"(xr[25]), [x26] "=&a"(xr[26]), [x27] "=&a"(xr[27]), [x28] "=&a"(xr[28]), [x29] "=&a"(xr[29]), [x30] "=&a"(xr[30]), [x31] "=&a"(xr[31])
-                     : [xb0] "v"(xb[0]), [xb1] "v"(xb[1]), [xb2] "v"(xb[2]), [xb3] "v"(xb[3]), [xb4] "v"(xb[4]), [xb5] "v"(xb[5]), [xb6] "v"(xb[6]), [xb7] "v"(xb[7])
-                       , [xo1] "n"(XS), [xo2] "n"(2 * XS), [xo3] "n"(3 * XS)
-                     : "memory");
-    }
-}
-
 __device__ __forceinline__ void ch_layernorm_pack8(f32x16 (&acc)[8], unsigned tab_lane, int off_a, int off_b, int off_add,
                                                    float eps, v4i (&b8)[8]) {
     float s = 0.f;
@@ -355,6 +258,19 @@
 #define CH_PRE_B_5 CH_PRE_BO
 #define CH_PRE_B_6 CH_PRE_BE
 #define CH_PRE_B_7 CH_PRE_BO
+#ifdef CH_EXP_NO_BARRIER
+#define CH_PRE_BEN(N, M0OFF) "s_waitcnt vmcnt(" #N ")\n\t" CH_PRE_BO(M0OFF)
+#else
+#define CH_PRE_BEN(N, M0OFF) "s_waitcnt vmcnt(" #N ")\n\ts_barrier\n\ts_add_u32 m0, %[m0w], " CH_STR(M0OFF) "\n\ts_waitcnt lgkmcnt(0)\n\t"
+#endif
+#define CH_PRE_S1_0(M0OFF) CH_PRE_BEN(41, M0OFF)
+#define CH_PRE_S1_1 CH_PRE_BO
+#define CH_PRE_S1_2(M0OFF) CH_PRE_BEN(33, M0OFF)
+#define CH_PRE_S1_3 CH_PRE_BO
+#define CH_PRE_S1_4(M0OFF) CH_PRE_BEN(25, M0OFF)
+#define CH_PRE_S1_5 CH_PRE_BO
+#define CH_PRE_S1_6 CH_PRE_BE
+#define CH_PRE_S1_7 CH_PRE_BO
 #ifdef CH_EXP_NO_DMA
 #define CH_DMA0(SOFF) "v_add_u32 %[tv], " CH_STR(SOFF) ", %[vo]\n\t"
 #define CH_DMA1 ""
@@ -378,26 +294,6 @@
                  CH_MF "%[c], %[f7], %[b7], %[c]\n\t" D3 POST                                                  \
                  : [c] CIO CC(acc), [n0] "=&v"(Fn[0]), [n1] "=&v"(Fn[1]), [n2] "=&v"(Fn[2]), [n3] "=&v"(Fn[3]), \
                    [n4] "=&v"(Fn[4]), [n5] "=&v"(Fn[5]), [n6] "=&v"(Fn[6]), [n7] "=&v"(Fn[7]), [tv] "=&v"(tv)  \
-                 : [f0] "v"(Fc[0]), [f1] "v"(Fc[1]), [f2] "v"(Fc[2]), [f3] "v"(Fc[3]), [f4] "v"(Fc[4]),        \
-                   [f5] "v"(Fc[5]), [f6] "v"(Fc[6]), [f7] "v"(Fc[7]), [b0] "v"(B[(BO) + 0]), [b1] "v"(B[(BO) + 1]), \
-                   [b2] "v"(B[(BO) + 2]), [b3] "v"(B[(BO) + 3]), [b4] "v"(B[(BO) + 4]), [b5] "v"(B[(BO) + 5]), \
-                   [b6] "v"(B[(BO) + 6]), [b7] "v"(B[(BO) + 7]), [ra] "v"(RA), [m0w] "s"(m0_wave), [vo] "v"(voff), \
-                   [sb] "s"(SB)                                                                                \
-                 : "memory", "scc")
-#define CH_BLK1A(K, acc, Fc, B, BO, Fn, RA, RK, PRE, D0, D1, D2, D3, SB, POST)                                 \
-    asm volatile(PRE                                                                                           \
-                 CH_MF "%[c" #K "], %[f0], %[b0], %[c" #K "]\n\t" CH_RD2(n0, n1, (RK) + 0)                       \
-                 CH_MF "%[c" #K "], %[f1], %[b1], %[c" #K "]\n\t" CH_RD2(n2, n3, (RK) + 2)                       \
-                 CH_MF "%[c" #K "], %[f2], %[b2], %[c" #K "]\n\t" CH_RD2(n4, n5, (RK) + 4)                       \
-                 CH_MF "%[c" #K "], %[f3], %[b3], %[c" #K "]\n\t" CH_RD2(n6, n7, (RK) + 6)                       \
-                 CH_MF "%[c" #K "], %[f4], %[b4], %[c" #K "]\n\t" D0                                           \
-                 CH_MF "%[c" #K "], %[f5], %[b5], %[c" #K "]\n\t" D1                                           \
-                 CH_MF "%[c" #K "], %[f6], %[b6], %[c" #K "]\n\t" D2                                           \
-                 CH_MF "%[c" #K "], %[f7], %[b7], %[c" #K "]\n\t" D3 POST                                      \
-                 : [c0] "+a"(acc[0]), [c1] "+a"(acc[1]), [c2] "+a"(acc[2]), [c3] "+a"(acc[3]), [c4] "+a"(acc[4]), \
-                   [c5] "+a"(acc[5]), [c6] "+a"(acc[6]), [c7] "+a"(acc[7]), [n0] "=&v"(Fn[0]), [n1] "=&v"(Fn[1]), \
-                   [n2] "=&v"(Fn[2]), [n3] "=&v"(Fn[3]), [n4] "=&v"(Fn[4]), [n5] "=&v"(Fn[5]), [n6] "=&v"(Fn[6]), \
-                   [n7] "=&v"(Fn[7]), [tv] "=&v"(tv)                                                           \
                  : [f0] "v"(Fc[0]), [f1] "v"(Fc[1]), [f2] "v"(Fc[2]), [f3] "v"(Fc[3]), [f4] "v"(Fc[4]),        \
                    [f5] "v"(Fc[5]), [f6] "v"(Fc[6]), [f7] "v"(Fc[7]), [b0] "v"(B[(BO) + 0]), [b1] "v"(B[(BO) + 1]), \
                    [b2] "v"(B[(BO) + 2]), [b3] "v"(B[(BO) + 3]), [b4] "v"(B[(BO) + 4]), [b5] "v"(B[(BO) + 5]), \
@@ -468,6 +364,149 @@
     X(4, ra1, 8, ra1, 16, 0xC000, 0xC000, sb_next)   X(5, ra1, 24, ra1, 32, 0x10000, 0x10000, sb_next)         \
     X(6, ra1, 40, ra1, 48, 0x14000, 0x14000, sb_next) X(7, ra1, 56, ra0, 0, 0x18000, 0x18000, sb_next)
 
+#define CH_PRO_X(NT, R0, R1, R2, R3)                                                                           \
+    "global_load_dwordx4 a[" R0 "], %[vx" #NT "], %[sx0]\n\t"                                                   \
+    "global_load_dwordx4 a[" R1 "], %[vx" #NT "], %[sx1]\n\t"                                                   \
+    "global_load_dwordx4 a[" R2 "], %[vx" #NT "], %[sx2]\n\t"                                                   \
+    "global_load_dwordx4 a[" R3 "], %[vx" #NT "], %[sx3]\n\t"
+#define CH_PRO_X0 CH_PRO_X(0, "0:3", "4:7", "8:11", "12:15")
+#define CH_PRO_X1 CH_PRO_X(1, "16:19", "20:23", "24:27", "28:31")
+#define CH_PRO_X2 CH_PRO_X(2, "32:35", "36:39", "40:43", "44:47")
+#define CH_PRO_X3 CH_PRO_X(3, "48:51", "52:55", "56:59", "60:63")
+#define CH_PRO_X4 CH_PRO_X(4, "64:67", "68:71", "72:75", "76:79")
+#define CH_PRO_X5 CH_PRO_X(5, "80:83", "84:87", "88:91", "92:95")
+#define CH_PRO_X6 CH_PRO_X(6, "96:99", "100:103", "104:107", "108:111")
+#define CH_PRO_X7 CH_PRO_X(7, "112:115", "116:119", "120:123", "124:127")
+#define CH_PRO_C(Q, C0, C1, C2, C3)                                                                            \
+    "global_load_dwordx4 %[" #C0 "], %[vc" #Q "], %[sc0]\n\t"                                                   \
+    "global_load_dwordx4 %[" #C1 "], %[vc" #Q "], %[sc1]\n\t"                                                   \
+    "global_load_dwordx4 %[" #C2 "], %[vc" #Q "], %[sc2]\n\t"                                                   \
+    "global_load_dwordx4 %[" #C3 "], %[vc" #Q "], %[sc3]\n\t"
+#define CH_PRO_U(U)                                                                                            \
+    "s_add_u32 m0, %[m0w], " CH_STR((U) * 0x4000) "\n\t"                                                       \
+    "v_add_u32 %[tv], " CH_STR((U) * 0x4000) ", %[vo]\n\t"                                                     \
+    "global_load_lds_dwordx4 %[tv], %[sb]\n\t"                                                                 \
+    "global_load_lds_dwordx4 %[tv], %[sb] offset:1024\n\t"                                                     \
+    "global_load_lds_dwordx4 %[tv], %[sb] offset:2048\n\t"                                                     \
+    "global_load_lds_dwordx4 %[tv], %[sb] offset:3072\n\t"
+#define CH_PRO_T                                                                                               \
+    "s_mov_b32 m0, %[tm0]\n\t"                                                                                 \
+    "v_add_u32 %[tv], 4096, %[tvo]\n\t"                                                                        \
+    "global_load_lds_dwordx4 %[tvo], %[stab]\n\t"                                                              \
+    "global_load_lds_dwordx4 %[tvo], %[stab] offset:1024\n\t"                                                  \
+    "global_load_lds_dwordx4 %[tvo], %[stab] offset:2048\n\t"                                                  \
+    "global_load_lds_dwordx4 %[tvo], %[stab] offset:3072\n\t"                                                  \
+    "s_add_u32 m0, %[tm0], 4096\n\t"                                                                           \
+    "s_nop 0\n\t"                                                                                              \
+    "global_load_lds_dwordx4 %[tv], %[stab]\n\t"
+#define CH_PRO_ACC_OUT                                                                                         \
+    "={a[0:15]}"(acc[0]), "={a[16:31]}"(acc[1]), "={a[32:47]}"(acc[2]), "={a[48:63]}"(acc[3]), "={a[64:79]}"(acc[4]),  \
+    "={a[80:95]}"(acc[5]), "={a[96:111]}"(acc[6]), "={a[112:127]}"(acc[7])
+#define CH_PRO_X_IN                                                                                            \
+    [vx0] "v"(a.vx[0]), [vx1] "v"(a.vx[1]), [vx2] "v"(a.vx[2]), [vx3] "v"(a.vx[3]), [vx4] "v"(a.vx[4]), [vx5] "v"(a.vx[5]),  \
+    [vx6] "v"(a.vx[6]), [vx7] "v"(a.vx[7]), [sx0] "s"(a.sx[0]), [sx1] "s"(a.sx[1]), [sx2] "s"(a.sx[2]), [sx3] "s"(a.sx[3])
+#define CH_PRO_RING_IN [vo] "v"(a.voff), [sb] "s"(a.sb), [m0w] "s"(a.m0_wave)
+#define CH_PRO_TAB_IN [tvo] "v"(a.tvo), [stab] "s"(a.stab), [tm0] "s"(a.tm0)
+
+struct ChPrologue {
+    unsigned vx[8], vc[4];
+    const char *sx[4], *sc[4];
+    unsigned voff, m0_wave;
+    const uint4 *sb, *sb_next;
+    unsigned tvo, tm0;
+    const float* stab;
+    unsigned ra0, ra1;
+};
+
+#define CH_S1_MF(K, F, i, B) CH_MF "%[a" #K "], %[" #F #i "], %[" #B "], %[a" #K "]\n\t"
+#ifdef CH_EXP_NO_READ
+#define CH_S1_RD2(N, i, j, RA, K) ""
+#else
+#define CH_S1_RD2(N, i, j, RA, K) "ds_read_b128 %[" #N #i "], %[" #RA "] offset:" CH_STR((K) * 1024) "\n\t"    \
+                                  "ds_read_b128 %[" #N #j "], %[" #RA "] offset:" CH_STR(((K) + 1) * 1024) "\n\t"
+#endif
+#ifdef CH_EXP_NO_DMA
+#define CH_S1_DMA0(SOFF, SB) "v_add_u32 %[tv], " CH_STR(SOFF) ", %[vo]\n\t"
+#define CH_S1_DMA(SB, OFF) ""
+#else
+#define CH_S1_DMA0(SOFF, SB) "v_add_u32 %[tv], " CH_STR(SOFF) ", %[vo]\n\tglobal_load_lds_dwordx4 %[tv], %[" #SB "]\n\t"
+#define CH_S1_DMA(SB, OFF) "global_load_lds_dwordx4 %[tv], %[" #SB "] offset:" #OFF "\n\t"
+#endif
+#define CH_S1_A(K, RA, RK)                                                                                     \
+    CH_PRE_A                                                                                                   \
+    CH_S1_MF(K, fa, 0, c0) CH_S1_RD2(fb, 0, 1, RA, (RK) + 0)                                                   \
+    CH_S1_MF(K, fa, 1, c1) CH_S1_RD2(fb, 2, 3, RA, (RK) + 2)                                                   \
+    CH_S1_MF(K, fa, 2, c2) CH_S1_RD2(fb, 4, 5, RA, (RK) + 4)                                                   \
+    CH_S1_MF(K, fa, 3, c3) CH_S1_RD2(fb, 6, 7, RA, (RK) + 6)                                                   \
+    CH_S1_MF(K, fa, 4, c4) CH_S1_MF(K, fa, 5, c5) CH_S1_MF(K, fa, 6, c6) CH_S1_MF(K, fa, 7, c7)
+#define CH_S1_B(K, RA, RK, PRE, SOFF, SB)                                                                      \
+    PRE                                                                                                        \
+    CH_S1_MF(K, fb, 0, c8) CH_S1_RD2(fa, 0, 1, RA, (RK) + 0)                                                   \
+    CH_S1_MF(K, fb, 1, c9) CH_S1_RD2(fa, 2, 3, RA, (RK) + 2)                                                   \
+    CH_S1_MF(K, fb, 2, c10) CH_S1_RD2(fa, 4, 5, RA, (RK) + 4)                                                  \
+    CH_S1_MF(K, fb, 3, c11) CH_S1_RD2(fa, 6, 7, RA, (RK) + 6)                                                  \
+    CH_S1_MF(K, fb, 4, c12) CH_S1_DMA0(SOFF, SB)                                                               \
+    CH_S1_MF(K, fb, 5, c13) CH_S1_DMA(SB, 1024)                                                                \
+    CH_S1_MF(K, fb, 6, c14) CH_S1_DMA(SB, 2048)                                                                \
+    CH_S1_MF(K, fb, 7, c15) CH_S1_DMA(SB, 3072)
+#define CH_S1_POS(k, RA_A, RK_A, RA_B, RK_B, M0OFF, SOFF, SB)                                                  \
+    CH_S1_A(k, RA_A, RK_A) CH_S1_B(k, RA_B, RK_B, CH_PRE_S1_##k(M0OFF), SOFF, SB)
+
+__device__ __forceinline__ void ch_s1(f32x16 (&acc)[8], bf16x8 (&bop)[16], bf16x8 (&Fa)[8], bf16x8 (&Fb)[8], const ChPrologue& a,
+                                      unsigned long long& t1, unsigned long long& t2) {
+    unsigned tv;
+    asm volatile(CH_PRO_U(0)
+                 CH_PRO_C(0, c0, c1, c2, c3) CH_PRO_C(1, c4, c5, c6, c7) CH_PRO_C(2, c8, c9, c10, c11) CH_PRO_C(3, c12, c13, c14, c15)
+                 CH_PRO_X0
+                 CH_PRO_X1 CH_PRO_U(1) CH_PRO_X2 CH_PRO_U(2)
+                 CH_PRO_X3 CH_PRO_U(3) CH_PRO_X4 CH_PRO_U(4)
+                 CH_PRO_X5 CH_PRO_U(5) CH_PRO_X6 CH_PRO_U(6)
+                 CH_PRO_X7 CH_PRO_T
+                 "s_waitcnt vmcnt(57)\n\t"
+                 "s_memtime %[t1]\n\t"
+                 "s_barrier\n\t"
+                 "s_memtime %[t2]\n\t"
+                 CH_S1_RD2(fa, 0, 1, ra0, 0) CH_S1_RD2(fa, 2, 3, ra0, 2) CH_S1_RD2(fa, 4, 5, ra0, 4) CH_S1_RD2(fa, 6, 7, ra0, 6)
+                 CH_POSITIONS(CH_S1_POS)
+                 "s_waitcnt lgkmcnt(0)\n\t"
+                 CH_DRAIN
+                 : [a0] "={a[0:15]}"(acc[0]), [a1] "={a[16:31]}"(acc[1]), [a2] "={a[32:47]}"(acc[2]), [a3] "={a[48:63]}"(acc[3]),
+                   [a4] "={a[64:79]}"(acc[4]), [a5] "={a[80:95]}"(acc[5]), [a6] "={a[96:111]}"(acc[6]), [a7] "={a[112:127]}"(acc[7]),
+                   [c0] "=&v"(bop[0]), [c1] "=&v"(bop[1]), [c2] "=&v"(bop[2]), [c3] "=&v"(bop[3]), [c4] "=&v"(bop[4]),
+                   [c5] "=&v"(bop[5]), [c6] "=&v"(bop[6]), [c7] "=&v"(bop[7]), [c8] "=&v"(bop[8]), [c9] "=&v"(bop[9]),
+                   [c10] "=&v"(bop[10]), [c11] "=&v"(bop[11]), [c12] "=&v"(bop[12]), [c13] "=&v"(bop[13]), [c14] "=&v"(bop[14]),
+                   [c15] "=&v"(bop[15]), [fa0] "=&v"(Fa[0]), [fa1] "=&v"(Fa[1]), [fa2] "=&v"(Fa[2]), [fa3] "=&v"(Fa[3]),
+                   [fa4] "=&v"(Fa[4]), [fa5] "=&v"(Fa[5]), [fa6] "=&v"(Fa[6]), [fa7] "=&v"(Fa[7]), [fb0] "=&v"(Fb[0]),
+                   [fb1] "=&v"(Fb[1]), [fb2] "=&v"(Fb[2]), [fb3] "=&v"(Fb[3]), [fb4] "=&v"(Fb[4]), [fb5] "=&v"(Fb[5]),
+                   [fb6] "=&v"(Fb[6]), [fb7] "=&v"(Fb[7]), [tv] "=&v"(tv), [t1] "=&s"(t1), [t2] "=&s"(t2)
+                 : CH_PRO_X_IN, [vc0] "v"(a.vc[0]), [vc1] "v"(a.vc[1]), [vc2] "v"(a.vc[2]), [vc3] "v"(a.vc[3]), [sc0] "s"(a.sc[0]),
+                   [sc1] "s"(a.sc[1]), [sc2] "s"(a.sc[2]), [sc3] "s"(a.sc[3]), CH_PRO_RING_IN, CH_PRO_TAB_IN,
+                   [sb_cur] "s"(a.sb), [sb_next] "s"(a.sb_next), [ra0] "v"(a.ra0), [ra1] "v"(a.ra1)
+                 : "memory", "scc");
+}
+
+template <bool RING>
+__device__ __forceinline__ void ch_prologue_x(f32x16 (&acc)[8], const ChPrologue& a) {
+    unsigned tv;
+    if constexpr (RING) {
+        asm volatile(CH_PRO_X0 CH_PRO_X1 CH_PRO_X2 CH_PRO_X3 CH_PRO_X4 CH_PRO_X5 CH_PRO_X6 CH_PRO_X7
+                     CH_PRO_T
+                     CH_PRO_U(0) CH_PRO_U(1) CH_PRO_U(2) CH_PRO_U(3) CH_PRO_U(4) CH_PRO_U(5) CH_PRO_U(6)
+                     "s_waitcnt vmcnt(24)"
+                     : CH_PRO_ACC_OUT, [tv] "=&v"(tv)
+                     : CH_PRO_X_IN, CH_PRO_RING_IN, CH_PRO_TAB_IN
+                     : "memory", "scc");
+    } else {
+        asm volatile(CH_PRO_X0 CH_PRO_X1 CH_PRO_X2 CH_PRO_X3 CH_PRO_X4 CH_PRO_X5 CH_PRO_X6 CH_PRO_X7
+                     CH_PRO_T
+                     "s_waitcnt vmcnt(0)"
+                     : CH_PRO_ACC_OUT, [tv] "=&v"(tv)
+                     : CH_PRO_X_IN, CH_PRO_TAB_IN
+                     : "memory", "scc");
+    }
+}
+
+
 template <bool SWISH, bool F8>
 __global__ __launch_bounds__(256) void chain_kernel(ChainParams p) {
     extern __shared__ __attribute__((aligned(16))) unsigned char smem[];
@@ -496,90 +535,69 @@
         return p.wstream + (long long)g * 8 * 1024;
     };
 
-    f32x4 xr[32];
+    f32x16 acc[8];
     bf16x8 bop[16];
     const int rb = blockIdx.x * 4 + wave, nrb = (p.M + 31) >> 5;
-    {
-        const uint4* ts = reinterpret_cast<const uint4*>(p.tab) + 5 * wave * 64 + lane;
-#pragma unroll
-        for (int j = 0; j < 5; ++j) CH_DMA(ts + j * 64, smem + (5 * wave + j) * 1024);
-    }
-    if (NG > 0) {
-        const uint4* g0 = group_base(0);
-        for (int u = 0; u < CH_RING - 1; ++u) {
-            const uint4* src = g0 + ((long long)u * 16 + 4 * wave) * 64 + lane;
-            unsigned char* dst = ring + u * CH_UNIT_BYTES + 4 * wave * 1024;
-#pragma unroll
-            for (int j = 0; j < 4; ++j) CH_DMA(src + j * 64, dst + j * 1024);
-        }
-    }
-    {
-#ifdef CH_EXP_HOT_X
-        const float* xp = p.x + (long long)wave * 8192 + 4 * lane;
-#else
-        const float* xp = p.x_in_blk ? p.x + (long long)(rb < nrb ? rb : nrb - 1) * 8192 + 4 * lane
-                                     : p.x + (long long)mc * CH_D + 4 * half;
-#endif
-        const int step = p.x_in_blk ? 256 : 8;
-        const float* xb[8];
-#pragma unroll
-        for (int nt = 0; nt < 8; ++nt) xb[nt] = xp + step * 4 * nt;
-        const bf16* cp = !p.ctx ? nullptr
-                         : p.ctx_blk ? p.ctx + ((long long)(rb < nrb ? rb : nrb - 1) * 16 * 64 + lane) * 8
-                                     : p.ctx + (long long)mc * p.ldctx + 8 * half;
-        const int cstep = p.ctx_blk ? 512 : 16;
-        const bf16* cb[4];
-#pragma unroll
-        for (int q = 0; q < 4; ++q) cb[q] = cp + cstep * 4 * q;
-        if (!p.ctx) {
-            if (p.x_in_blk) ch_load_rows<1024, 32, false>(xr, bop, xb, cb);
-            else ch_load_rows<32, 32, false>(xr, bop, xb, cb);
-        } else if (p.x_in_blk) {
-            if (p.ctx_blk) ch_load_rows<1024, 1024, true>(xr, bop, xb, cb);
-            else ch_load_rows<1024, 32, true>(xr, bop, xb, cb);
-        } else {
-            if (p.ctx_blk) ch_load_rows<32, 1024, true>(xr, bop, xb, cb);
-            else ch_load_rows<32, 32, true>(xr, bop, xb, cb);
-        }
-    }
-
-    f32x16 acc[8];
-#pragma unroll
-    for (int nt = 0; nt < 8; ++nt)
-#pragma unroll
-        for (int g = 0; g < 4; ++g)
-#pragma unroll
-            for (int e = 0; e < 4; ++e) acc[nt][4 * g + e] = xr[4 * nt + g][e];
-    CH_STAMP(1)
-
     const unsigned ring_lds = (unsigned)(size_t)(__attribute__((address_space(3))) unsigned char*)ring;
     const unsigned ra0 = ring_lds + lane * 16, ra1 = ra0 + 4 * CH_UNIT_BYTES;
     const unsigned tab_lane = (unsigned)(size_t)(__attribute__((address_space(3))) unsigned char*)(smem + 16 * half);
     const unsigned voff = (unsigned)(lane * 16 + wave * 4096);
     const unsigned m0_wave = __builtin_amdgcn_readfirstlane(ring_lds + wave * 4096);
     unsigned tv = 0;
+    ChPrologue pro;
+    {
+        const int rbl = (rb < nrb ? rb : nrb - 1) - (int)blockIdx.x * 4, ml = mc - (int)blockIdx.x * 128;
+#ifdef CH_EXP_HOT_X
+        const char* xbase = reinterpret_cast<const char*>(p.x);
+        const unsigned xlane = (unsigned)(wave * 32768 + lane * 16), xs = 1024;
+#else
+        const char* xbase = reinterpret_cast<const char*>(p.x) + (long long)blockIdx.x * (128 * CH_D * 4);
+        const unsigned xlane = p.x_in_blk ? (unsigned)(rbl * 32768 + lane * 16) : (unsigned)(ml * (CH_D * 4) + 16 * half);
+        const unsigned xs = p.x_in_blk ? 1024 : 32;
+#endif
+#pragma unroll
+        for (int nt = 0; nt < 8; ++nt) pro.vx[nt] = xlane + 4 * xs * nt;
+#pragma unroll
+        for (int g = 0; g < 4; ++g) pro.sx[g] = xbase + g * xs;
+        if (p.ctx) {
+            const char* cbase = reinterpret_cast<const char*>(p.ctx) +
+                                (p.ctx_blk ? (long long)blockIdx.x * (4 * 16384) : (long long)blockIdx.x * 128 * p.ldctx * 2);
+            const unsigned clane = p.ctx_blk ? (unsigned)(rbl * 16384 + lane * 16) : (unsigned)(ml * p.ldctx * 2 + 16 * half);
+            const unsigned cs = p.ctx_blk ? 1024 : 32;
+#pragma unroll
+            for (int q = 0; q < 4; ++q) pro.vc[q] = clane + 4 * cs * q;
+#pragma unroll
+            for (int g = 0; g < 4; ++g) pro.sc[g] = cbase + g * cs;
+        }
+        pro.voff = voff;
+        pro.m0_wave = m0_wave;
+        pro.sb = NG > 0 ? group_base(0) : p.wstream;
+        pro.ra0 = ra0;
+        pro.ra1 = ra1;
+        pro.tvo = (unsigned)(lane * 16 + wave * 5120);
+        pro.tm0 = __builtin_amdgcn_readfirstlane((unsigned)(size_t)(__attribute__((address_space(3))) unsigned char*)smem + wave * 5120);
+        pro.stab = p.tab;
+    }
 
     bf16x8 Fa[8], Fb[8];
-    asm volatile("s_waitcnt vmcnt(0)\n\ts_barrier" ::: "memory");
-    CH_STAMP(2)
     int gpos = 0;
 
     if (p.ctx) {
-        const uint4* sb_cur = group_base(gpos);
-        const uint4* sb_next = group_base(gpos + 1);
-#define CH_S1(k, RA_A, RK_A, RA_B, RK_B, M0OFF, SOFF, SB)                                                     \
-        CH_BLK1A(k, acc, Fa, bop, 0, Fb, RA_A, RK_A, CH_PRE_A, "", "", "", "", SB, CH_NODRAIN);                \
-        CH_BLK1A(k, acc, Fb, bop, 8, Fa, RA_B, RK_B, CH_PRE_B_##k(M0OFF), CH_DMA0(SOFF), CH_DMA1, CH_DMA2, CH_DMA3, SB, CH_NODRAIN);
-        CH_READ8(Fa, ra0, 0);
-        CH_WAIT8(Fa);
-        asm volatile("s_nop 1" ::: "memory");
-        CH_POSITIONS(CH_S1)
-#undef CH_S1
-        CH_LAND_FRAGMENTS("");
-        asm volatile(CH_DRAIN : "+a"(acc[0]), "+a"(acc[1]), "+a"(acc[2]), "+a"(acc[3]), "+a"(acc[4]), "+a"(acc[5]),
-                     "+a"(acc[6]), "+a"(acc[7]) :: "memory");
+        unsigned long long t1, t2;
+        pro.sb_next = group_base(1);
+        ch_s1(acc, bop, Fa, Fb, pro, t1, t2);
+        if (p.stamps && (int)blockIdx.x == p.stamp_block && tid == 0) {
+            ch_stamps[1] = (long long)t1;
+            ch_stamps[2] = (long long)t2;
+        }
         ++gpos;
         ch_add_channel(acc, tab_lane, CT_BO);
+    } else {
+        if (NG > 0) ch_prologue_x<true>(acc, pro);
+        else ch_prologue_x<false>(acc, pro);
+        CH_STAMP(1)
+        asm volatile("s_barrier" ::: "memory");
+        CH_STAMP(2)
     }
     CH_STAMP(3)
 
@@ -950,6 +968,7 @@
     static const char* names[] = {"prologue issue", "x/ctx landed + acc", "first unit visible", "S1 out-proj", "LN1 + b2",
                                   "S3 ffn loop", "S4 x store", "LNn", "S5 tail", "drain"};
     for (int i = 1; i < 10; ++i) fprintf(stderr, "[chain stamps] %-20s %8lld ticks\n", names[i], h[i] - h[i - 1]);
+    fprintf(stderr, "[chain stamps] %-20s %8lld ticks\n", "prologue + S1", h[3] - h[0]);
     fprintf(stderr, "[chain stamps] total %lld ticks (s_memtime)\n", h[9] - h[0]);
     fprintf(stderr, "[chain stamps] wall %.2f us (s_memrealtime) -> %.0f MHz\n", (h[11] - h[10]) / 100.0,
             (double)(h[9] - h[0]) / ((h[11] - h[10]) / 100.0));
diff --git a/cassnat_asr_public_amd/csrc/ops.hip b/cassnat_asr_public_amd/csrc/ops.hip
--- a/cassnat_asr_public_amd/csrc/ops.hip
+++ b/cassnat_asr_public_amd/csrc/ops.hip
@@ -1040,6 +1040,10 @@
         cn_set_error("cn_op_chain: the e4m3 feed-forward form (x_mode bit 32) needs d_ff % 256 == 0 and the ReLU activation");
         return -1;
     }
+    if ((x_mode & 64) && ctx_dev && ldctx != 256) {
+        cn_set_error("cn_op_chain: a blocked ctx (x_mode bit 64) has ldctx == 256");
+        return -1;
+    }
     const size_t units = chain_stream_units(ctx_dev != nullptr, dff, tail_n, f8);
     std::vector<uint16_t> hs((units + 7) * (CHAIN_UNIT_BYTES / 2));
     std::vector<float> ht(CHAIN_TAB_FLOATS + 4);
@@ -1069,6 +1073,7 @@
     a.store_x = (x_mode & 4) == 0;
     a.swish = (x_mode & 8) != 0;
     a.out_blocked = (x_mode & 16) != 0;
+    a.ctx_blocked = (x_mode & 64) != 0;
     a.f8 = f8;
     a.f8_q = f8 ? reinterpret_cast<const int*>(dt + CHAIN_TAB_FLOATS) : nullptr;
     int rc = launch_chain(a, (hipStream_t)stream);
```
